# utiasASRL/dICP

Hardware: AMD Instinct MI355X
Metric: ICP cloud-iterations/sec (fwd+bwd), B=256x16384-pt clouds per GPU (higher is better)
Workload: dtype f32

## Files before the change

### dicp_amd/_lib.py

```python
import ctypes
import os
import subprocess
import threading

_HERE = os.path.dirname(os.path.abspath(__file__))
_ROOT = os.path.dirname(_HERE)
LIB_PATH = os.environ.get("DICP_HIP_LIB") or os.path.join(_HERE, "libdicp_hip.so")
SOURCES = [os.path.join(_HERE, "csrc", f) for f in ("dicp_kernels.hip", "knn_f16.hip", "dicp_call.hip", "normals.hip", "voxel.hip", "knn_points.hip", "fps.hip", "ball_query.hip", "knn_grid.hip", "group.hip", "inverse.hip", "knn_det.hip", "normals_det.hip", "filter.hip")]
HEADERS = ([os.path.join(_HERE, "csrc", f) for f in ("dicp_math.h", "dicp_common.h", "dicp_internal.h", "dicp_fill.h", "dicp_normals.h", "dicp_voxel.h", "dicp_topk.h", "dicp_fps.h", "dicp_ball.h", "dicp_gridknn.h", "kernels_grid.h", "kernels_grid_plan.h", "dicp_group.h", "dicp_group_launch.h", "dicp_inverse.h", "dicp_knn_det.h", "kernels_normals.h", "dicp_normals_det.h", "dicp_filter.h")]
           + [os.path.join(_HERE, "csrc", "kernels_%s.h" % f) for f in ("setup", "search", "setup_sort", "rows", "accumulate", "backward", "soft_svd", "host")]
           + [os.path.join(_ROOT, "include", "dicp_hip.h")])

F32, F64 = 0, 1
PT2PT, PT2PL = 0, 1
LOSS_NONE, LOSS_HUBER, LOSS_CAUCHY, LOSS_TRIM = 0, 1, 2, 3
KNN_AUTO, KNN_VALU, KNN_MFMA, KNN_SWEEP, KNN_GUMBEL = 0, 1, 2, 3, 4
FPS_AUTO, FPS_RESIDENT, FPS_STREAMED = 0, 1, 2
POOL_SUM, POOL_MEAN, POOL_MAX = 0, 1, 2
NACC_PAD, NBWD_PAD, KAB_SAVE = 32, 16, 40
PAIR_SHARDS = 64
ABI_VERSION = 11
_ERRORS = {1: "null pointer", 2: "bad shape/stride", 3: "unsupported dtype", 4: "bad enum value", 5: "misaligned buffer"}

vp, i32, i64, f64 = ctypes.c_void_p, ctypes.c_int32, ctypes.c_int64, ctypes.c_double


class WeightParams(ctypes.Structure):
    _fields_ = [("mode", i32), ("trim_on", i32), ("differentiable", i32), ("loss", i32),
                ("trim_dist", f64), ("tanh_k", f64), ("loss_delta", f64), ("match_thresh", f64)]


class StepIO(ctypes.Structure):
    _fields_ = [("partials", vp), ("nblk", i32), ("iter", i32), ("dim", i32), ("const_iter", i32),
                ("tolerance", f64), ("rows_per_point", i32), ("n", i32),
                ("pose_in", vp), ("pose_out", vp), ("delta", vp), ("delta_stride", i64),
                ("cost", vp), ("cost_prev", vp), ("cost_stride", i64), ("areg", vp), ("alive", vp), ("alive_out", vp),
                ("converged", vp), ("iterations", vp), ("matched_ratio", vp), ("n_start", vp),
                ("n_matched", vp), ("w_cur", vp), ("w_prev", vp), ("w_stride", i64), ("n_not_converged", vp),
                ("frame", vp), ("pose_search_out", vp), ("rmax", vp), ("dcum", vp), ("dcum_stride", i64), ("cert_cloud", vp),
                ("cert_qu", vp), ("cert_units", i32), ("glist_cap", i32), ("glist", vp), ("gcount", vp), ("cert_scount", vp), ("cert_slist", vp), ("w_copied", i32)]


class SearchBuffers(ctypes.Structure):
    _fields_ = [("knn_variant", i32), ("m_pad", i32), ("tgt4", vp), ("tperm", vp), ("qorder", vp), ("bucket", vp), ("brange", vp), ("nbkt", i32), ("pairs", vp), ("frame", vp), ("poses", vp),
                ("tgt_sorted", vp), ("tgt_sorted_stride", i32), ("gumbel", vp), ("first_done", i32), ("tgt_f16", vp), ("form", vp), ("form_default", i32), ("form_plan", vp)]


class CertBuffers(ctypes.Structure):
    _fields_ = [("q", vp), ("qu", vp), ("set", vp), ("count", vp), ("rmax", vp), ("dcum", vp), ("reset", i32), ("cloud", vp), ("nbr", vp), ("gdirty", vp), ("pend", vp), ("glist", vp),
                ("gcount", vp), ("slist", vp), ("scount", vp), ("cm", vp)]


class HistoryBuffers(ctypes.Structure):
    _fields_ = [("per_iter", i32), ("spos", vp), ("poses", vp), ("deltas", vp), ("costs", vp), ("areg", vp), ("alive", vp), ("idx", vp), ("w", vp), ("w_iter", i64), ("w_stride", i64),
                ("w_prev0", vp), ("spos_prev_chunk", vp), ("spos_floor", i32), ("spos_of", vp), ("spos_of_from", i32)]


class BwdBuffers(ctypes.Structure):
    _fields_ = [("spos_ref", vp), ("gts_far", vp), ("overwrite", i32), ("skip", vp), ("mref", vp), ("live", vp), ("skip_eps", f64), ("tail_from", i32), ("tail_partials", vp),
                ("tail_arrive", vp), ("det_far_row", vp), ("det_far_val", vp)]


class LoopBuffers(ctypes.Structure):
    _fields_ = [("abi", i32), ("src", vp), ("tgt", vp), ("w_init", vp), ("c", i32), ("K", i32), ("converged", vp), ("iterations", vp), ("matched_ratio", vp), ("n_start", vp), ("n_matched", vp),
                ("partials", vp), ("counters", vp), ("counters_host", vp), ("counters_tag", i32), ("events", vp), ("src_rows", vp), ("tgt_rows", vp),
                ("search", SearchBuffers), ("cert", CertBuffers), ("hist", HistoryBuffers), ("bwd", BwdBuffers)]

    def __init__(self, **kw):
        super().__init__(abi=ABI_VERSION)
        subs = (self, self.search, self.cert, self.hist, self.bwd)
        where = LoopBuffers._KW
        for k, v in kw.items():
            if v is not None:
                i, f = where[k]
                setattr(subs[i], f, v)


LoopBuffers._KW = dict([(f[0], (0, f[0])) for f in LoopBuffers._fields_[:-4]] +
                       [(g + "_" + f[0], (i + 1, f[0])) for i, (g, cls) in enumerate((("search", SearchBuffers), ("cert", CertBuffers), ("hist", HistoryBuffers), ("bwd", BwdBuffers)))
                        for f in cls._fields_])


class GumbelLoop(ctypes.Structure):
    _fields_ = [("U", vp), ("seeds", vp), ("eps", f64), ("tau", f64), ("ps_t", vp), ("nbr", vp), ("lse", vp), ("g_nbr", vp), ("g_ps", vp)]


MAX_SEGMENTS = 16
CERT_OFF_FOR_GOOD = 1 << 20


class SegmentPlan(ctypes.Structure):
    _fields_ = [("nseg", i32), ("k0", i32 * MAX_SEGMENTS), ("k1", i32 * MAX_SEGMENTS), ("new_order", i32 * MAX_SEGMENTS),
                ("cert_from", i32), ("pad0", i32), ("order", vp * MAX_SEGMENTS), ("keys", vp), ("cert_q", vp), ("cert_qu", vp), ("cert_count", vp), ("cert_cloud", vp), ("cert_set", vp),
                ("cert_nbr", vp), ("cert_gdirty", vp), ("cert_pend", vp), ("cert_cm", vp), ("cert_glist", vp), ("cert_gcount", vp), ("cert_slist", vp), ("cert_scount", vp)]


class Call(ctypes.Structure):
    _fields_ = [("src", vp), ("tgt", vp), ("T_init", vp), ("w0", vp), ("N", i32), ("n", i32), ("m", i32), ("c", i32), ("K", i32), ("dim", i32), ("need_grad", i32),
                ("n_resort", i32), ("resort", i32 * MAX_SEGMENTS), ("flags", i32), ("directions", i32), ("quantum", f64), ("tolerance", f64), ("workspace", vp), ("results", vp), ("T_out", vp), ("pc_out", vp)]


_sz = ctypes.c_size_t


class CallLayout(ctypes.Structure):
    _fields_ = ([(k, _sz) for k in ("total", "zeroed", "results_total", "results_zeroed", "T", "pc", "deltas", "weights", "costs", "converged", "iterations", "matched_ratio", "pairs", "n_matched", "counters",
                                    "poses", "poses_search", "alive", "areg", "n_start", "partials", "tgs4", "tperm", "bucket", "brange", "keys", "tgt_sorted", "scratch",
                                    "scratch_bytes", "frame", "pose_s", "orders", "spos")]
                + [("n_orders", i32), ("m_pad", i32), ("nblk", i32), ("pad0", i32)])


class CallGrads(ctypes.Structure):
    _fields_ = [("gT", vp), ("gsrc", vp), ("gtgt", vp), ("gT0", vp), ("gw", vp), ("workspace", vp), ("skip_eps", f64), ("tail_from", i32), ("pad0", i32), ("live_host", vp)]


class CallBackwardLayout(ctypes.Structure):
    _fields_ = ([(k, _sz) for k in ("total", "zeroed", "live", "arrive", "mref", "decisions", "far", "gpose", "gtmp", "src_s", "w_s", "gsrc_s", "gw_s", "slab", "gs", "gb",
                                    "partials", "tail_partials", "spos_ref")] + [("nblk_w", i32), ("pad0", i32)])


class LoopBackwardIn(ctypes.Structure):
    _fields_ = ([(k, vp) for k in ("src", "tgt_sorted", "w0", "tperm", "qorder", "spos", "poses", "deltas", "areg", "alive", "src_rows", "tgt_rows", "spos_of")]
                + [(k, i32) for k in ("N", "n", "m", "c", "K", "K_cap", "m_pad", "dim", "knn_variant", "spos_of_from")]
                + [(k, vp) for k in ("src_s", "w_s", "spos_ref")])


class KabschCall(ctypes.Structure):
    _fields_ = [("src", vp), ("tgt", vp), ("T_start", vp), ("w0", vp), ("N", i32), ("n", i32), ("m", i32), ("c", i32), ("K", i32), ("trim_on", i32), ("directions", i32), ("pad0", i32),
                ("trim_dist", f64), ("quantum", f64), ("tolerance", f64), ("workspace", vp), ("T_out", vp), ("pc_out", vp)]


class KabschCallLayout(ctypes.Structure):
    _fields_ = ([(k, _sz) for k in ("total", "zeroed", "costs", "iterations", "pairs", "counters", "frame", "keys", "tperm", "bucket", "brange", "tgs4", "scratch", "scratch_bytes",
                                    "pose", "pose_search", "pose_used", "partials", "save", "idx", "rows_live", "orders", "gpose", "gacc")] + [("m_pad", i32), ("nblk", i32)])


class KabschCallGrads(ctypes.Structure):
    _fields_ = [("gT", vp), ("gsrc", vp), ("gtgt", vp), ("gw", vp)]


CALL_FIRST_SEARCH, CALL_NO_SMALL_LOOP, CALL_NBKT = 1, 2, 1024


class KabschBuffers(ctypes.Structure):
    _fields_ = [("src", vp), ("tgt", vp), ("w_init", vp), ("c", i32), ("K", i32), ("knn_variant", i32), ("m_pad", i32), ("tgt4", vp), ("tperm", vp),
                ("qorder", vp), ("bucket", vp), ("brange", vp), ("nbkt", i32), ("pad0", i32), ("pairs", vp), ("frame", vp), ("pose", vp),
                ("pose_search", vp), ("pose_used", vp), ("idx", vp), ("partials", vp), ("save", vp), ("costs", vp), ("iterations", vp),
                ("rows_live", vp), ("tgt_rows", vp), ("counters", vp), ("tgt_f16", vp)]


_SIGNATURES = {
    "dicp_abi_version": ([], ctypes.c_int),
    "dicp_copy": ([vp, vp, ctypes.c_size_t, vp], ctypes.c_int),
    "dicp_zero": ([vp, ctypes.c_size_t, vp], ctypes.c_int),
    "dicp_padded_targets": ([i32], ctypes.c_int),
    "dicp_accumulate_blocks": ([i32], ctypes.c_int),
    "dicp_pack_target": ([i32, vp, i32, vp, vp, i32, i32, vp, i32, vp], ctypes.c_int),
    "dicp_search_frame": ([i32, vp, i32, vp, i32, i32, f64, i32, vp, vp, i32, vp, vp, vp], ctypes.c_int),
    "dicp_knn_f16_bytes": ([i32, i32], ctypes.c_size_t),
    "dicp_knn_f16_pack": ([vp, vp, i32, i32, i32, vp, vp], ctypes.c_int),
    "dicp_knn_f16_probe": ([vp, vp, vp, vp, vp, vp, i32, i32, i32, i32, vp, vp], ctypes.c_int),
    "dicp_knn": ([i32, vp, vp, vp, vp, vp, i32, i32, i32, i32, vp, i32, vp, vp], ctypes.c_int),
    "dicp_knn_sweep": ([i32, vp, vp, vp, vp, vp, vp, vp, i32, vp, vp, i32, i32, i32, i32, vp, vp, vp, i32, vp, vp, vp, i32, vp], ctypes.c_int),
    "dicp_window_blocks": ([i32, i32, i32], ctypes.c_int),
    "dicp_window_rows": ([i32], ctypes.c_int),
    "dicp_bwd_tail_max_blocks": ([i32], ctypes.c_int),
    "dicp_sweep_sort_scratch_bytes": ([i32, i32, i32], ctypes.c_size_t),
    "dicp_sweep_sort": ([i32, vp, i32, vp, vp, i32, i32, i32, vp, vp, i32, vp, vp, vp, ctypes.c_size_t, vp], ctypes.c_int),
    "dicp_sweep_build": ([i32, vp, i32, vp, vp, vp, i32, i32, i32, vp, vp, i32, vp], ctypes.c_int),
    "dicp_sweep_setup": ([i32, vp, i32, vp, i32, i32, i32, f64, i32, vp, vp, vp, i32, vp, vp, vp, ctypes.c_size_t, vp, vp, i32, vp, vp, i32, vp, vp, vp, vp], ctypes.c_int),
    "dicp_query_order": ([i32, vp, vp, vp, i32, i32, i32, vp, vp, vp, vp, i32, vp, i32, vp, vp, i32, vp, vp, vp], ctypes.c_int),
    "dicp_query_reorder": ([i32, vp, vp, vp, vp, vp, i32, i32, i32, vp, i32, vp, vp, i32, vp, vp, vp], ctypes.c_int),
    "dicp_query_keys": ([i32, vp, vp, i32, i32, vp, vp], ctypes.c_int),
    "dicp_loop_init": ([i32, vp, vp, ctypes.c_double, i32, i32, i32, vp, vp, vp, vp, vp, vp, vp, vp, i32, vp], ctypes.c_int),
    "dicp_search_pose": ([i32, vp, vp, i32, vp, vp], ctypes.c_int),
    "dicp_loop_finish": ([i32, vp, vp, vp, vp, i32, i32, vp, vp, vp, vp], ctypes.c_int),
    "dicp_accumulate_bwd_window": ([i32, ctypes.POINTER(WeightParams), vp, vp, i32, vp, vp, vp, vp, vp, vp, vp, vp, vp, i32, i32, i32, vp, vp, vp, vp, vp, i32, vp], ctypes.c_int),
    "dicp_resolve_matches": ([vp, vp, i32, vp, i32, i32, vp, vp], ctypes.c_int),
    "dicp_match_order_scratch_bytes": ([i32, i32, i32], ctypes.c_size_t),
    "dicp_match_order": ([i32, vp, vp, i32, i32, vp, ctypes.c_size_t, vp, vp], ctypes.c_int),
    "dicp_window_reduce": ([i32, vp, vp, vp, vp, vp, vp, i32, i32, i32, i32, i32, vp, i32, i32, vp], ctypes.c_int),
    "dicp_permute_add_rows": ([i32, vp, vp, i32, i32, i32, i32, i32, i32, vp, i32, i32, vp], ctypes.c_int),
    "dicp_pose_grad_in": ([i32, vp, vp, i32, vp], ctypes.c_int),
    "dicp_pose_grad_out": ([i32, vp, vp, i32, vp, i32, vp], ctypes.c_int),
    "dicp_permute_rows": ([i32, vp, vp, i32, i32, i32, i32, i32, i32, vp, i32, i32, vp], ctypes.c_int),
    "dicp_gather_rows": ([i32, vp, vp, i32, i32, i32, i32, vp, vp], ctypes.c_int),
    "dicp_scatter_add_rows": ([i32, vp, vp, i32, i32, i32, i32, vp, vp], ctypes.c_int),
    "dicp_pack_list": ([i32, vp, vp, vp, i32, i32, i32, vp, vp, vp], ctypes.c_int),
    "dicp_unpack_list": ([i32, vp, vp, vp, vp, i32, i32, i32, i32, vp], ctypes.c_int),
    "dicp_accumulate": ([i32, ctypes.POINTER(WeightParams), vp, vp, i32, vp, vp, vp, vp, vp, i32, i32, i32, vp, vp, i64, vp], ctypes.c_int),
    "dicp_step": ([i32, ctypes.POINTER(StepIO), i32, vp], ctypes.c_int),
    "dicp_icp_forward": ([i32, ctypes.POINTER(WeightParams), ctypes.POINTER(LoopBuffers), i32, i32, i32, i32, i32, f64, i32, i32, vp], ctypes.c_int),
    "dicp_icp_forward_plan": ([i32, ctypes.POINTER(WeightParams), ctypes.POINTER(LoopBuffers), ctypes.POINTER(SegmentPlan), i32, i32, i32, i32, i32, f64, vp], ctypes.c_int),
    "dicp_icp_backward": ([i32, ctypes.POINTER(WeightParams), ctypes.POINTER(LoopBuffers), i32, i32, i32, i32, vp, vp, i32, vp, vp, vp, vp, vp, vp, i32, i32, vp], ctypes.c_int),
    "dicp_step_bwd": ([i32, vp, vp, i32, i32, vp, vp, i64, vp, vp, vp, vp, i32, vp], ctypes.c_int),
    "dicp_accumulate_bwd": ([i32, ctypes.POINTER(WeightParams), vp, vp, i32, vp, vp, vp, vp, vp, vp, vp, i32, i32, i32, vp, vp, vp, vp, vp], ctypes.c_int),
    "dicp_gumbel_nn": ([i32, vp, vp, i32, vp, ctypes.c_uint32, f64, f64, i32, i32, i32, vp, vp, vp], ctypes.c_int),
    "dicp_gumbel_nn_bwd": ([i32, vp, vp, i32, vp, ctypes.c_uint32, f64, f64, vp, vp, vp, i32, i32, i32, vp, vp, vp], ctypes.c_int),
    "dicp_kabsch_accumulate": ([i32, vp, vp, i32, vp, vp, vp, i32, f64, vp, i32, i32, i32, vp, vp], ctypes.c_int),
    "dicp_kabsch_step": ([i32, vp, i32, vp, vp, vp, i32, vp], ctypes.c_int),
    "dicp_kabsch_step_bwd": ([i32, vp, vp, vp, i32, vp], ctypes.c_int),
    "dicp_kabsch_forward": ([i32, ctypes.POINTER(KabschBuffers), i32, i32, i32, i32, f64, i32, f64, i32, i32, vp], ctypes.c_int),
    "dicp_kabsch_bwd": ([i32, vp, vp, i32, vp, vp, vp, i32, f64, vp, vp, i32, i32, i32, vp, vp, vp, vp], ctypes.c_int),
    "dicp_transform_points": ([i32, vp, vp, vp, i32, i32, vp], ctypes.c_int),
    "dicp_transform_points_bwd": ([i32, vp, vp, vp, vp, vp, i32, i32, vp], ctypes.c_int),
    "dicp_loss_weight": ([i32, i32, i32, f64, f64, vp, i64, i32, vp, vp], ctypes.c_int),
    "dicp_loss_weight_bwd": ([i32, i32, i32, f64, f64, vp, vp, i64, i32, vp, vp], ctypes.c_int),
    "dicp_call_plan": ([i32, ctypes.POINTER(Call), ctypes.POINTER(CallLayout)], ctypes.c_int),
    "dicp_call_forward": ([i32, ctypes.POINTER(WeightParams), ctypes.POINTER(Call), vp], ctypes.c_int),
    "dicp_call_backward_plan": ([i32, ctypes.POINTER(WeightParams), ctypes.POINTER(Call), i32, i32, ctypes.POINTER(CallBackwardLayout)], ctypes.c_int),
    "dicp_call_backward": ([i32, ctypes.POINTER(WeightParams), ctypes.POINTER(Call), ctypes.POINTER(CallGrads), vp], ctypes.c_int),
    "dicp_loop_backward_plan": ([i32, ctypes.POINTER(WeightParams), ctypes.POINTER(LoopBackwardIn), i32, i32, ctypes.POINTER(CallBackwardLayout)], ctypes.c_int),
    "dicp_loop_backward": ([i32, ctypes.POINTER(WeightParams), ctypes.POINTER(LoopBackwardIn), ctypes.POINTER(CallGrads), vp], ctypes.c_int),
    "dicp_loop_backward_prepare": ([i32, ctypes.POINTER(LoopBackwardIn), vp, vp, vp, vp], ctypes.c_int),
    "dicp_kabsch_call_plan": ([i32, ctypes.POINTER(KabschCall), ctypes.POINTER(KabschCallLayout)], ctypes.c_int),
    "dicp_kabsch_call_forward": ([i32, ctypes.POINTER(KabschCall), vp], ctypes.c_int),
    "dicp_kabsch_call_backward": ([i32, ctypes.POINTER(KabschCall), ctypes.POINTER(KabschCallGrads), vp], ctypes.c_int),
    "dicp_normals_workspace_bytes": ([i32, i32, i32, i32, i32, i32], ctypes.c_size_t),
    "dicp_normals_forward": ([i32, vp, i32, vp, i32, i32, i32, vp, i32, vp, vp, vp, vp, ctypes.c_size_t, vp, vp], ctypes.c_int),
    "dicp_normals_backward": ([i32, vp, vp, vp, i32, vp, i32, i32, i32, i32, vp, vp, vp, ctypes.c_size_t, vp], ctypes.c_int),
    "dicp_normals_grid_workspace_bytes": ([i32, i32, i32, i32, i32, i32], ctypes.c_size_t),
    "dicp_normals_grid_forward": ([i32, vp, i32, vp, i32, i32, i32, vp, i32, vp, vp, vp, vp, ctypes.c_size_t, vp, vp, vp], ctypes.c_int),
    "dicp_normals_grid_backward": ([i32, vp, vp, vp, i32, i32, i32, i32, i32, vp, vp, vp, ctypes.c_size_t, vp], ctypes.c_int),
    "dicp_voxel_workspace_bytes": ([i32, i32, i32, i32], ctypes.c_size_t),
    "dicp_voxel_count": ([i32, vp, i32, vp, i32, i32, f64, f64, f64, vp, i32, i32, vp, vp, ctypes.c_size_t, vp], ctypes.c_int),
    "dicp_voxel_reduce": ([i32, vp, i32, i32, i32, i32, vp, ctypes.c_size_t, vp, vp, vp, vp], ctypes.c_int),
    "dicp_voxel_backward": ([i32, vp, vp, vp, i32, i32, i32, i32, vp, vp], ctypes.c_int),
    "dicp_knn_points_workspace_bytes": ([i32, i32, i32, i32, i32, i32], ctypes.c_size_t),
    "dicp_knn_points": ([i32, vp, vp, vp, i32, vp, vp, vp, vp, i32, i32, i32, vp, vp, vp, ctypes.c_size_t, vp, vp], ctypes.c_int),
    "dicp_knn_points_backward": ([i32, vp, vp, vp, vp, i32, i32, vp, vp, i32, i32, i32, i32, vp, vp, vp, vp, ctypes.c_size_t, vp], ctypes.c_int),
    "dicp_fps_geometry": ([i32, ctypes.POINTER(i32), ctypes.POINTER(i32), ctypes.POINTER(i32)], None),
    "dicp_fps_workspace_bytes": ([i32, i32, i32, i32, i32], ctypes.c_size_t),
    "dicp_fps_forward": ([i32, vp, i32, vp, vp, i32, i32, i32, i32, vp, vp, vp, vp, vp, ctypes.c_size_t, vp], ctypes.c_int),
    "dicp_fps_backward": ([i32, vp, vp, i32, i32, i32, i32, vp, vp], ctypes.c_int),
    "dicp_ball_grid_slots": ([i32], ctypes.c_int),
    "dicp_ball_plan_bytes": ([], ctypes.c_int),
    "dicp_ball_grid_build": ([i32, vp, i32, vp, i32, i32, vp, vp, vp, vp, vp, vp, vp], ctypes.c_int),
    "dicp_ball_query_workspace_bytes": ([i32, i32, i32, i32], ctypes.c_size_t),
    "dicp_ball_query": ([i32, vp, i32, i32, vp, vp, vp, vp, vp, vp, i32, i32, i32, vp, vp, vp, vp, ctypes.c_size_t, vp, vp], ctypes.c_int),
    "dicp_ball_query_backward": ([i32, vp, vp, i32, i32, vp, vp, i32, i32, i32, i32, vp, vp, vp, vp], ctypes.c_int),
    "dicp_knn_grid_build": ([i32, vp, i32, vp, i32, i32, vp, vp, vp, vp, vp], ctypes.c_int),
    "dicp_knn_grid_query": ([i32, vp, i32, i32, vp, vp, vp, vp, vp, vp, i32, i32, i32, vp, vp, vp, ctypes.c_size_t, vp, vp, vp], ctypes.c_int),
    "dicp_group_forward": ([i32, vp, vp, i32, vp, vp, i32, i32, i32, i32, i32, i32, vp, vp], ctypes.c_int),
    "dicp_group_backward": ([i32, vp, vp, i32, vp, i32, i32, i32, i32, i32, i32, vp, vp, vp], ctypes.c_int),
    "dicp_interpolate_forward": ([i32, vp, vp, i32, vp, vp, f64, i32, i32, i32, i32, i32, vp, vp], ctypes.c_int),
    "dicp_interpolate_backward": ([i32, vp, vp, vp, vp, i32, vp, vp, f64, i32, i32, i32, i32, i32, vp, vp, vp], ctypes.c_int),
    "dicp_pool_forward": ([i32, vp, vp, i32, vp, i32, i32, i32, i32, i32, i32, vp, vp, vp, vp], ctypes.c_int),
    "dicp_pool_backward": ([i32, vp, vp, i32, vp, i32, vp, vp, i32, i32, i32, i32, i32, vp, vp], ctypes.c_int),
    "dicp_invert_neighbors_workspace_bytes": ([i32, i32, i32, i32], ctypes.c_size_t),
    "dicp_invert_neighbors": ([vp, i32, vp, i32, i32, i32, i32, vp, vp, vp, ctypes.c_size_t, vp], ctypes.c_int),
    "dicp_group_backward_det": ([i32, vp, vp, i32, vp, i32, i32, i32, i32, i32, vp, vp, vp, vp], ctypes.c_int),
    "dicp_pool_backward_det": ([i32, vp, vp, i32, vp, i32, vp, vp, i32, i32, i32, i32, i32, vp, vp, vp, vp], ctypes.c_int),
    "dicp_interpolate_backward_det": ([i32, vp, vp, i32, vp, vp, f64, i32, i32, i32, i32, i32, vp, vp, vp, vp], ctypes.c_int),
    "dicp_knn_backward_y_det": ([i32, vp, vp, vp, vp, i32, i32, vp, i32, i32, i32, i32, vp, vp, vp, vp], ctypes.c_int),
    "dicp_normals_backward_records": ([i32, i32, vp, vp, vp, i32, vp, i32, i32, i32, i32, vp, ctypes.c_size_t, vp, vp, vp], ctypes.c_int),
    "dicp_normals_gather_det": ([i32, vp, vp, i32, vp, i32, i32, i32, i32, vp, vp, vp, vp], ctypes.c_int),
    "dicp_select_workspace_bytes": ([i32, i32], ctypes.c_size_t),
    "dicp_select_rows": ([i32, vp, i32, vp, vp, i32, i32, vp, vp, vp, vp, vp, ctypes.c_size_t, vp], ctypes.c_int),
    "dicp_select_rows_backward": ([i32, vp, vp, i32, i32, i32, vp, vp], ctypes.c_int),
    "dicp_outlier_workspace_bytes": ([i32, i32], ctypes.c_size_t),
    "dicp_outlier_stats": ([i32, vp, vp, vp, i32, i32, i32, f64, vp, vp, vp, vp, ctypes.c_size_t, vp], ctypes.c_int),
}
EXPORTS = tuple(_SIGNATURES)

_lib = None
_lock = threading.Lock()


FLAGS = ["-O3", "-std=c++17", "--offload-arch=gfx950", "-fPIC", "-ffp-contract=on", "-mllvm", "-amdgpu-mfma-vgpr-form", "-Wall", "-Wno-unused-function"]


def build(force=False, verbose=False):
    hdr_time = max(os.path.getmtime(p) for p in HEADERS + [os.path.abspath(__file__)])
    hipcc = os.environ.get("HIPCC", "/opt/rocm/bin/hipcc")
    objdir = os.path.join(_HERE, "csrc", "_obj")
    os.makedirs(objdir, exist_ok=True)
    jobs = []
    for src in SOURCES:
        obj = os.path.join(objdir, os.path.splitext(os.path.basename(src))[0] + ".o")
        if force or not os.path.exists(obj) or os.path.getmtime(obj) < max(os.path.getmtime(src), hdr_time):
            jobs.append((src, obj))
    objs = [os.path.join(objdir, os.path.splitext(os.path.basename(src))[0] + ".o") for src in SOURCES]
    if not jobs and os.path.exists(LIB_PATH) and os.path.getmtime(LIB_PATH) >= max(os.path.getmtime(o) for o in objs):
        return LIB_PATH

    def compile_one(job):
        cmd = [hipcc] + FLAGS + ["-I", os.path.join(_ROOT, "include"), "-c", "-o", job[1] + ".tmp", job[0]]
        if verbose:
            print(" ".join(cmd))
        subprocess.check_call(cmd)
        os.replace(job[1] + ".tmp", job[1])
    if jobs:
        from concurrent.futures import ThreadPoolExecutor
        with ThreadPoolExecutor(max_workers=min(len(jobs), 4)) as pool:
            list(pool.map(compile_one, jobs))
    cmd = [hipcc, "--offload-arch=gfx950", "-shared", "-fPIC", "-o", LIB_PATH + ".tmp"] + objs
    if verbose:
        print(" ".join(cmd))
    subprocess.check_call(cmd)
    os.replace(LIB_PATH + ".tmp", LIB_PATH)
    return LIB_PATH


def load():
    global _lib
    if _lib is not None:
        return _lib
    import torch
    with _lock:
        if _lib is None:
            if not os.path.exists(LIB_PATH):
                raise RuntimeError(
                    "dicp_amd: %s is missing -- build it with `python -c 'import __graft_entry__ as g; g.build()'` "
                    "(hipcc --offload-arch=gfx950).  There is no CPU fallback." % LIB_PATH)
            lib = ctypes.CDLL(LIB_PATH)
            for name, (args, res) in _SIGNATURES.items():
                fn = getattr(lib, name)
                fn.argtypes = args
                fn.restype = res
            if lib.dicp_abi_version() != ABI_VERSION:
                raise RuntimeError("dicp_amd: libdicp_hip.so ABI version mismatch; rebuild it")
            _lib = lib
    return _lib
# ... 20 lines not shown
```

### dicp_amd/_ops.py

```python
import os
import ctypes

import torch

from . import _lib

_DT = {torch.float32: _lib.F32, torch.float64: _lib.F64}
SWEEP_MIN_TARGETS = 2048
SWEEP_MIN_QUERIES = 256
F16_SWEEP = True
F16_SWEEP_MIN_QUERIES = 2 * 256 * 1024
F16_SWEEP_MIN_TARGETS = 16384
FORM_PLAN_ITERS = 6
FORM_TILES_MOVING = 32
F16_SWEEP_STATIC_TARGETS = 32768
F16_SWEEP_ADAPTIVE = os.environ.get("DICP_F16_ADAPTIVE", "1") != "0"
FORM_TILES = 12
SWEEP_MIN_PAIRS = 1e8


def auto_knn_kind(N, n, m):
    big = m >= SWEEP_MIN_TARGETS and n >= SWEEP_MIN_QUERIES and float(N) * n * m >= SWEEP_MIN_PAIRS
    return _lib.KNN_SWEEP if big else _lib.KNN_VALU
_LOSS = {None: _lib.LOSS_NONE, "huber": _lib.LOSS_HUBER, "cauchy": _lib.LOSS_CAUCHY, "trim": _lib.LOSS_TRIM}
# ... 19 lines not shown


def _stream():
    if _raw_stream is not None and _raw_device is not None:
        return ctypes.c_void_p(_raw_stream(_raw_device()))
    return ctypes.c_void_p(torch.cuda.current_stream().cuda_stream)


def _p(t):
    return ctypes.c_void_p(t.data_ptr()) if t is not None else None


def _workspace(nbytes, device):
    buf = torch.empty(nbytes + 256, dtype=torch.uint8, device=device)
    return buf[(-buf.data_ptr()) % 256:]


class _NoSwitch:
    def __enter__(self):
        return None

    def __exit__(self, *exc):
        return False


_NO_SWITCH = _NoSwitch()


def _on(device):
    if _raw_device is not None and device.index is not None and _raw_device() == device.index:
        return _NO_SWITCH
    return torch.cuda.device(device)


def padded_targets(m):
    return _lib.load().dicp_padded_targets(int(m))


def accumulate_blocks(n):
    return _lib.load().dicp_accumulate_blocks(int(n))


CENTER_QUANTUM = 16.0
FRAME_DIRECTIONS = True


def search_frame(tgt, quantum=None, tgt_rows=None, directions=None, src=None, T_init=None, src_rows=None):
    require_device(tgt, "search_frame")
    N, m, c = tgt.shape
    out = torch.empty((N, 12), dtype=tgt.dtype, device=tgt.device)
    with_q = src is not None and T_init is not None
    if with_q:
        src, T_init = src.contiguous(), T_init.contiguous()
    with _on(tgt.device):
        _lib.check(_lib.load().dicp_search_frame(_DT[tgt.dtype], _p(tgt), c, _p(tgt_rows), N, m, CENTER_QUANTUM if quantum is None else float(quantum),
                                                 int(FRAME_DIRECTIONS if directions is None else directions),
                                                 _p(src) if with_q else None, _p(src_rows) if with_q else None, int(src.shape[1]) if with_q else 0,
                                                 _p(T_init) if with_q else None, _p(out), _stream()), "dicp_search_frame")
    return out


def search_pose(pose, frame, N=None):
    if pose is None:
        if frame is not None:
            return frame.clone()
        pose = torch.zeros((N, 12))
        pose[:, 0] = pose[:, 4] = pose[:, 8] = 1.0
        return pose
    if frame is None:
        return pose
    n = pose.shape[0]
    Q, t = frame[:, :9].reshape(n, 3, 3), frame[:, 9:]
    out = torch.empty_like(pose)
    out[:, :9] = torch.matmul(Q, pose[:, :9].reshape(n, 3, 3)).reshape(n, 9)
    out[:, 9:] = torch.matmul(Q, pose[:, 9:, None]).squeeze(-1) + t
    return out


def pack_target(tgt, frame=None, tgt_rows=None):
    require_device(tgt, "pack_target")
    tgt = tgt.contiguous()
    N, m, c = tgt.shape
    m_pad = padded_targets(m)
    out = torch.empty((N, m_pad, 4), dtype=tgt.dtype, device=tgt.device)
    with _on(tgt.device):
        _lib.check(_lib.load().dicp_pack_target(_DT[tgt.dtype], _p(tgt), c, _p(frame), _p(tgt_rows), N, m, _p(out), m_pad, _stream()),
                   "dicp_pack_target")
    return out


def f16_image(tgt4, m, tgt_rows=None):
    require_device(tgt4, "f16_image")
    if tgt4.dtype != torch.float32:
        raise TypeError("dicp_amd.f16_image: the matrix-core search is float32 only")
    lib = _lib.load()
    N, m_pad, _ = tgt4.shape
    img = torch.empty((int(lib.dicp_knn_f16_bytes(N, m_pad)),), dtype=torch.uint8, device=tgt4.device)
    with _on(tgt4.device):
        _lib.check(lib.dicp_knn_f16_pack(_p(tgt4), _p(tgt_rows), N, int(m), m_pad, _p(img), _stream()), "dicp_knn_f16_pack")
    return img


def f16_counters(image, N, m_pad):
    m_img = (int(m_pad) + 511) // 512 * 512
    meta = image[N * m_img * 32:N * m_img * 32 + N * 320].view(torch.int32).view(N, 80)
    return int(meta[:, 6].sum().item()), int(meta[:, 7].sum().item())


def knn(src, pose, tgt4, m, variant=_lib.KNN_AUTO, out=None, src_rows=None, tgt_rows=None, image=None):
    require_device(src, "knn")
    N, n, _ = src.shape
    idx = out if out is not None else torch.empty((N, n), dtype=torch.int32, device=src.device)
    if (variant & 0xff) == _lib.KNN_MFMA and image is None and src.dtype == torch.float32:
        image = f16_image(tgt4, m, tgt_rows)
    with _on(src.device):
        _lib.check(_lib.load().dicp_knn(_DT[src.dtype], _p(src), _p(pose), _p(tgt4), _p(src_rows), _p(tgt_rows), N, n, m, tgt4.shape[1],
                                        _p(idx), variant, _p(image), _stream()), "dicp_knn")
    return idx


class SweepIndex:
    NBKT = 1024

    def __init__(self, tgt, sorted_rows=False, frame=None, tgt_rows=None, first_order=None, first_search=False, tally=True):
        require_device(tgt, "SweepIndex")
        tgt = tgt.contiguous()
        N, m, c = tgt.shape
        self.m = m
        self.frame, self.tgt_rows = frame, tgt_rows
        lib = _lib.load()
        dev, dt = tgt.device, tgt.dtype
        m_pad = lib.dicp_padded_targets(m)
        self.tgs4 = torch.empty((N, m_pad, 4), dtype=dt, device=dev)
        self.tperm = torch.empty((N, m_pad), dtype=torch.int32, device=dev)
        self.bucket = torch.empty((N, self.NBKT + 1), dtype=torch.int32, device=dev)
        self.brange = torch.empty((N, 2), dtype=dt, device=dev)
        self.keys = torch.empty((N, m_pad), dtype=dt, device=dev)
        self.row_stride = c
        self.tgt_s = torch.empty((N, m_pad, self.row_stride), dtype=dt, device=dev) if sorted_rows else None
        nbytes = int(lib.dicp_sweep_sort_scratch_bytes(_DT[dt], N, m_pad))
        scratch = torch.empty((nbytes,), dtype=torch.uint8, device=dev) if nbytes else None
        self.first = None
        self.pair_shards = torch.zeros((_lib.PAIR_SHARDS,), dtype=torch.int64, device=dev)
        self.img16 = None
        want_img = (bool(F16_SWEEP) and dt == torch.float32 and first_order is not None and float(N) * first_order[0].shape[1] >= F16_SWEEP_MIN_QUERIES
                    and m >= F16_SWEEP_MIN_TARGETS)
        self.form_default = int(m >= F16_SWEEP_MIN_TARGETS)
        self.form0 = None
        if first_order is not None:
            source, T_init, src_rows = first_order
            self.frame = torch.empty((N, 12), dtype=dt, device=dev)
            pose_s = torch.empty((N, 12), dtype=dt, device=dev)
            qorder = torch.empty((N, source.shape[1]), dtype=torch.int32, device=dev)
            with _on(dev):
                _lib.check(lib.dicp_sweep_setup(_DT[dt], _p(tgt), c, _p(tgt_rows), N, m, m_pad, CENTER_QUANTUM, int(FRAME_DIRECTIONS), _p(self.frame), _p(self.keys), _p(self.tperm),
                                                self.NBKT, _p(self.bucket), _p(self.brange), _p(scratch), nbytes, _p(self.tgs4), _p(self.tgt_s), self.row_stride,
                                                _p(source), _p(src_rows), source.shape[1], _p(T_init), _p(pose_s), _p(qorder), _stream()), "dicp_sweep_setup")
            if want_img:
                self.img16 = f16_image(self.tgs4, m, tgt_rows)
            spos0 = None
            if first_search:
                spos0 = torch.empty((N, source.shape[1]), dtype=torch.int32, device=dev)
                if tally and F16_SWEEP_ADAPTIVE and dt == torch.float32 and float(N) * source.shape[1] >= F16_SWEEP_MIN_QUERIES and bool(F16_SWEEP):
                    self.form0 = torch.zeros((N,), dtype=torch.int32, device=dev)
                with _on(dev):
                    _lib.check(lib.dicp_knn_sweep(_DT[dt], _p(source), _p(pose_s), _p(self.tgs4), _p(self.tperm), _p(qorder), _p(self.bucket), _p(self.brange), self.NBKT,
                                                  _p(src_rows), _p(tgt_rows), N, source.shape[1], m, m_pad, None, _p(spos0), _p(self.pair_shards), 0,
                                                  _p(self.img16) if (self.form_default or not F16_SWEEP_ADAPTIVE) else None, None, _p(self.form0), self.form_default, _stream()), "dicp_knn_sweep")
            self.first = (source, T_init, qorder, spos0)
            return
        with _on(dev):
            _lib.check(lib.dicp_sweep_sort(_DT[dt], _p(tgt), c, _p(frame), _p(tgt_rows), N, m, m_pad, _p(self.keys), _p(self.tperm), self.NBKT,
                                           _p(self.bucket), _p(self.brange), _p(scratch), nbytes, _stream()), "dicp_sweep_sort")
            _lib.check(lib.dicp_sweep_build(_DT[dt], _p(tgt), c, _p(frame), _p(tgt_rows), _p(self.tperm), N, m, m_pad,
                                            _p(self.tgs4), _p(self.tgt_s), self.row_stride, _stream()), "dicp_sweep_build")

    @property
    def pairs(self):
        return self.pair_shards.sum()

    def query_order(self, src, pose, exact=False, w=None, copies=False, reproducible=False, spos_prev=None, src_rows=None, pose_prev=None, order_prev=None):
        N, n, _ = src.shape
        lib = _lib.load()
        with _on(src.device):
            if not exact and pose is not None and pose_prev is not None and order_prev is not None and not copies and spos_prev is None:
                qorder = torch.empty((N, n), dtype=torch.int32, device=src.device)
                _lib.check(lib.dicp_query_reorder(_DT[src.dtype], _p(src), _p(pose), _p(pose_prev), _p(order_prev), _p(self.brange), self.NBKT, N, n, _p(qorder),
                                                  self.tgs4.shape[1], _p(self.keys), _p(self.bucket), self.m, _p(src_rows), _p(self.tgt_rows), _stream()), "dicp_query_reorder")
                return qorder
            if not exact:
                qorder = torch.empty((N, n), dtype=torch.int32, device=src.device)
                _lib.check(lib.dicp_query_order(_DT[src.dtype], _p(src), _p(pose), _p(self.brange), self.NBKT, N, n, _p(qorder),
                                                None, None, None, int(reproducible), _p(spos_prev), self.tgs4.shape[1],
                                                _p(self.keys), _p(self.bucket), self.m, _p(src_rows), _p(self.tgt_rows), _stream()),
                           "dicp_query_order")
                if copies:
                    return qorder, _gather_rows_raw(src, qorder), (_gather_rows_raw(w.unsqueeze(-1), qorder).squeeze(-1) if w is not None else None)
                return qorder
            assert src_rows is None, "exact query order: dense batches only (a test / tuning aid)"
            keys = torch.empty((N, n), dtype=src.dtype, device=src.device)
            _lib.check(lib.dicp_query_keys(_DT[src.dtype], _p(src), _p(pose), N, n, _p(keys), _stream()), "dicp_query_keys")
        qorder = torch.argsort(keys, dim=1).to(torch.int32)
        if copies:
            return qorder, _gather_rows_raw(src, qorder), (_gather_rows_raw(w.unsqueeze(-1), qorder).squeeze(-1) if w is not None else None)
        return qorder

    def make_image(self):
        if self.img16 is None:
            self.img16 = f16_image(self.tgs4, self.m, self.tgt_rows)
        return self.img16

    def knn(self, src, pose, qorder=None, out=None, cfg=0, spos=None, src_rows=None, mfma=False):
        N, n, _ = src.shape
        idx = out if out is not None else torch.empty((N, n), dtype=torch.int32, device=src.device)
        with _on(src.device):
            _lib.check(_lib.load().dicp_knn_sweep(_DT[src.dtype], _p(src), _p(pose), _p(self.tgs4), _p(self.tperm), _p(qorder),
                                                  _p(self.bucket), _p(self.brange), self.NBKT, _p(src_rows), _p(self.tgt_rows), N, n, self.m, self.tgs4.shape[1],
                                                  _p(idx), _p(spos), _p(self.pair_shards), cfg, _p(self.make_image()) if mfma else None, None, None, 1, _stream()), "dicp_knn_sweep")
        return idx


class _GatherRows(torch.autograd.Function):

    @staticmethod
    def forward(ctx, y, idx):
        N, m, c = y.shape
        n = idx.shape[1]
        out = torch.empty((N, n, c), dtype=y.dtype, device=y.device)
        with _on(y.device):
            _lib.check(_lib.load().dicp_gather_rows(_DT[y.dtype], _p(y), _p(idx), N, n, m, c, _p(out), _stream()), "dicp_gather_rows")
        ctx.save_for_backward(idx)
        ctx.shape = (N, m, c)
        return out

    @staticmethod
    def backward(ctx, gout):
        (idx,) = ctx.saved_tensors
        N, m, c = ctx.shape
        gout = gout.contiguous()
        gy = torch.zeros((N, m, c), dtype=gout.dtype, device=gout.device)
        with _on(gout.device):
            _lib.check(_lib.load().dicp_scatter_add_rows(_DT[gout.dtype], _p(gout), _p(idx), N, idx.shape[1], m, c, _p(gy), _stream()),
                       "dicp_scatter_add_rows")
        return gy, None


def gather_rows(y, idx):
    return _GatherRows.apply(y.contiguous(), idx)


def _gather_rows_raw(y, idx):
    y = y.contiguous()
    N, m, c = y.shape
    k = idx.shape[1]
    out = torch.empty((N, k, c), dtype=y.dtype, device=y.device)
    with _on(y.device):
        _lib.check(_lib.load().dicp_gather_rows(_DT[y.dtype], _p(y), _p(idx), N, k, m, c, _p(out), _stream()), "dicp_gather_rows")
    return out


class _PackList(torch.autograd.Function):

    @staticmethod
    def forward(ctx, cols, pad, *clouds):
        lib = _lib.load()
        N, dev, dt = len(clouds), clouds[0].device, clouds[0].dtype
        for t in clouds:
            if not (t.is_cuda and t.device == dev and t.dtype == dt and t.dim() == 2 and t.shape[1] >= cols and (t.shape[0] <= 1 or t.stride(1) == 1) and t.stride(0) >= t.shape[1]):
                raise ValueError("pack_list: every cloud must be a 2-D %s tensor on %s with unit column stride and at least %d columns" % (dt, dev, cols))
        lens = [int(t.shape[0]) for t in clouds]
        n_max = max(lens)
        meta = torch.tensor([t.data_ptr() for t in clouds] + lens + [int(t.stride(0)) for t in clouds], dtype=torch.int64).to(dev)
        lens_d, strides_d = meta[N:2 * N].to(torch.int32), meta[2 * N:].to(torch.int32)
        out = torch.empty((N, n_max, cols), dtype=dt, device=dev)
        with _on(dev):
            _lib.check(lib.dicp_pack_list(_DT[dt], _p(meta), _p(lens_d), _p(strides_d), N, n_max, int(cols), _p(out), _p(pad), _stream()), "dicp_pack_list")
        ctx.geom = (cols, n_max, lens, [int(t.shape[1]) for t in clouds], dt, dev)
        ctx.lens_d = lens_d
        return out

    @staticmethod
    def backward(ctx, gout):
        cols, n_max, lens, widths, dt, dev = ctx.geom
        lib = _lib.load()
        N, es = len(lens), torch.empty((), dtype=dt).element_size()
        sizes = [l * c for l, c in zip(lens, widths)]
        offs = [0]
        for sz in sizes:
            offs.append(offs[-1] + sz)
        flat = torch.empty((offs[-1],), dtype=dt, device=dev)
        meta = torch.tensor([flat.data_ptr() + o * es for o in offs[:-1]] + widths, dtype=torch.int64).to(dev)
        strides_d = meta[N:].to(torch.int32)
        g = gout.contiguous()
        with _on(dev):
            _lib.check(lib.dicp_unpack_list(_DT[dt], _p(g), _p(meta), _p(ctx.lens_d), _p(strides_d), N, n_max, int(cols), max(widths), _stream()), "dicp_unpack_list")
        grads = tuple(flat[offs[i]:offs[i + 1]].view(lens[i], widths[i]) if ctx.needs_input_grad[2 + i] else None for i in range(N))
        return (None, None) + grads


def packable(clouds, widths):
    first = clouds[0]
    if not isinstance(first, torch.Tensor) or not first.is_cuda or first.dtype not in _DT:
        return False
    return all(isinstance(t, torch.Tensor) and t.is_cuda and t.dim() == 2 and t.shape[0] > 0 and t.shape[1] in widths and t.dtype == first.dtype
               and t.device == first.device and t.stride(1) == 1 for t in clouds)


def pack_list(clouds, cols, pad=None):
    return _PackList.apply(int(cols), pad, *clouds)


class _GumbelNN(torch.autograd.Function):
# ... 276 lines not shown
```

### dicp_amd/csrc/dicp_internal.h

```cpp
#pragma once
#include <stddef.h>
#include <stdint.h>

namespace dicp_tu {

constexpr int KNN_F16_META = 80;
constexpr int KNN_F16_STAGE_ROWS = 512;
inline int knn_f16_image_rows(int m_pad) { return (m_pad + KNN_F16_STAGE_ROWS - 1) / KNN_F16_STAGE_ROWS * KNN_F16_STAGE_ROWS; }
inline size_t knn_f16_image_bytes(int N, int m_pad) { return (size_t)N * ((size_t)knn_f16_image_rows(m_pad) * 32 + KNN_F16_META * 4 + (size_t)knn_f16_image_rows(m_pad) / 64 * 8); }
inline size_t knn_f16_meta_offset(int N, int m_pad) { return (size_t)N * knn_f16_image_rows(m_pad) * 32; }
inline size_t knn_f16_edges_offset(int N, int m_pad) { return knn_f16_meta_offset(N, m_pad) + (size_t)N * KNN_F16_META * 4; }
int knn_f16_pack(const void* rows4, const int32_t* tgt_rows, int N, int m_full, int m_pad, void* image, void* stream);
int knn_f16_probe(const void* src, const void* pose, const void* tgt4, const void* image, const int32_t* src_rows, const int32_t* tgt_rows,
                  int N, int n, int m, int m_pad, float* out, void* stream);
int knn_f16_brute(const void* src, const void* pose, const void* tgt4, void* image, const int32_t* src_rows, const int32_t* tgt_rows,
                  int N, int n, int m, int m_pad, int32_t* idx, void* stream);

int knn_f16_sweep(const void* src, const void* pose, const void* tgs4, void* image, const int32_t* tperm, const int32_t* qorder, const int32_t* bucket,
                  const void* brange, int nbkt, const int32_t* src_rows, const int32_t* tgt_rows, int N, int n, int m, int m_pad, int32_t* idx, int32_t* spos,
                  unsigned long long* pairs, const int32_t* form_in, int32_t* form_out, int form_tiles, int form_default, void* ev0, void* ev1, void* stream);

}
```

### dicp_amd/csrc/dicp_kernels.hip

```cpp
#include <hip/hip_runtime.h>
#include <hip/hip_ext.h>
#include <stdint.h>

#include "dicp_common.h"
#include "dicp_internal.h"
#include "dicp_fill.h"

namespace {

#include "kernels_setup.h"
#include "kernels_search.h"
#include "kernels_setup_sort.h"
#include "kernels_rows.h"
#include "kernels_accumulate.h"
#include "kernels_backward.h"
#include "kernels_soft_svd.h"
#include "kernels_host.h"

}

extern "C" {

int dicp_abi_version(void) { return DICP_ABI_VERSION; }
int dicp_copy(void* dst, const void* src, size_t bytes, void* stream) {
    if (!dst || !src) return DICP_ERR_NULL;
    if ((((uintptr_t)dst | (uintptr_t)src | bytes) & 3) != 0) return DICP_ERR_ALIGN;
    return dicp_fill::copy(dst, src, bytes, (hipStream_t)stream);
}
int dicp_zero(void* dst, size_t bytes, void* stream) {
    if (!dst) return DICP_ERR_NULL;
    if ((((uintptr_t)dst | bytes) & 3) != 0) return DICP_ERR_ALIGN;
    return dicp_fill::zero(dst, bytes, (hipStream_t)stream);
}
int dicp_padded_targets(int m) { return m <= 0 ? 0 : ((m + KNN_PAD - 1) / KNN_PAD) * KNN_PAD; }
int dicp_accumulate_blocks(int n) { return n <= 0 ? 0 : (n + ACC_PTS - 1) / ACC_PTS; }
int dicp_search_frame(int dtype, const void* tgt, int c, const int32_t* tgt_rows, int N, int m, double quantum, int directions,
                      const void* src, const int32_t* src_rows, int n, const void* T_init, void* frame, void* stream) {
    if (!tgt || !frame) return DICP_ERR_NULL;
    if (bad_dtype(dtype)) return DICP_ERR_DTYPE;
    if (N <= 0 || m <= 0 || c < 3 || !(quantum >= 0.0) || (src && T_init && n <= 0)) return DICP_ERR_SHAPE;
    if (!src || !T_init) { src = nullptr; T_init = nullptr; }
    begin_launch();
    if (dtype == DICP_F32) search_frame_kernel<float><<<N, CC_THREADS, 0, (hipStream_t)stream>>>((const float*)tgt, c, m, tgt_rows, quantum, directions, (float*)frame, (const float*)src, n, src_rows, (const float*)T_init);
    else                   search_frame_kernel<double><<<N, CC_THREADS, 0, (hipStream_t)stream>>>((const double*)tgt, c, m, tgt_rows, quantum, directions, (double*)frame, (const double*)src, n, src_rows, (const double*)T_init);
    return launch_status();
}

int dicp_pack_target(int dtype, const void* tgt, int c, const void* frame, const int32_t* tgt_rows, int N, int m, void* tgt4, int m_pad, void* stream) {
    if (!tgt || !tgt4) return DICP_ERR_NULL;
    if (bad_dtype(dtype)) return DICP_ERR_DTYPE;
    if (N <= 0 || m <= 0 || (c != 3 && c != 6) || m_pad != dicp_padded_targets(m)) return DICP_ERR_SHAPE;
    if ((uintptr_t)tgt4 % (dtype == DICP_F32 ? 16 : 32)) return DICP_ERR_ALIGN;
    hipStream_t st = (hipStream_t)stream;
    begin_launch();
    const int bpc = (int)blocks_for((size_t)m_pad);
    const unsigned g = grid_for(N, bpc);
    if (dtype == DICP_F32) pack_kernel<float><<<g, BLOCK, 0, st>>>((const float*)tgt, N, m, c, (float4*)tgt4, m_pad, bpc, (const float*)frame, tgt_rows);
    else                   pack_kernel<double><<<g, BLOCK, 0, st>>>((const double*)tgt, N, m, c, (double4*)tgt4, m_pad, bpc, (const double*)frame, tgt_rows);
    return launch_status();
}

size_t dicp_sweep_sort_scratch_bytes(int dtype, int N, int m_pad) {
    if (N <= 0 || m_pad <= 0 || (dtype == DICP_F32 && m_pad <= RS_MAX)) return 0;
    const size_t S = ((size_t)m_pad + GS_CHUNK - 1) / GS_CHUNK, passes = dtype == DICP_F32 ? 4 : 8;
    return (size_t)N * 2 * m_pad * ((dtype == DICP_F32 ? 4 : 8) + sizeof(int32_t)) + 256 + (S <= GS_MAX_CHUNKS ? passes * (size_t)N * S * S * 256 * sizeof(int32_t) : 0);
}

int dicp_sweep_sort(int dtype, const void* tgt, int c, const void* frame, const int32_t* tgt_rows, int N, int m, int m_pad, void* keys_sorted,
                    int32_t* tperm, int nbkt, int32_t* bucket, void* brange, void* scratch, size_t scratch_bytes, void* stream) {
    if (!tgt || !keys_sorted || !tperm || (bucket && !brange)) return DICP_ERR_NULL;
    if (bucket && nbkt <= 0) return DICP_ERR_SHAPE;
    if (bad_dtype(dtype)) return DICP_ERR_DTYPE;
    if (N <= 0 || m <= 0 || (c != 3 && c != 6) || m_pad != dicp_padded_targets(m)) return DICP_ERR_SHAPE;
    hipStream_t st = (hipStream_t)stream;
    if (dtype == DICP_F32 && m_pad <= RS_MAX) {
        begin_launch();
        sort_keys_kernel<<<N, RS_THREADS, 0, st>>>((const float*)tgt, c, N, m, m_pad, (float*)keys_sorted, tperm, nbkt, bucket, (float*)brange, (const float*)frame, tgt_rows);
        return launch_status();
    }
    if (!scratch || scratch_bytes < dicp_sweep_sort_scratch_bytes(dtype, N, m_pad)) return DICP_ERR_NULL;
    begin_launch();
    void* kb = (void*)(((uintptr_t)scratch + 15) & ~(uintptr_t)15);
    const int S = (m_pad + GS_CHUNK - 1) / GS_CHUNK;
    const bool several = S >= 2 && S <= GS_MAX_CHUNKS && (size_t)N * S <= 0x7fffffffu;
#define DICP_BIGSORT(T, KT) do { \
        int32_t* ib = (int32_t*)((KT*)kb + (size_t)N * 2 * m_pad); \
        int32_t* hist = ib + (size_t)N * 2 * m_pad; \
        if (several) { \
            constexpr int PASSES = (int)sizeof(KT); \
            sort_big_keys_kernel<T><<<N * S, GS_THREADS, 0, st>>>((const T*)tgt, c, m, m_pad, S, (const T*)frame, tgt_rows, (KT*)kb, ib, hist, N); \
            for (int p = 0; p + 1 < PASSES; ++p) sort_big_pass_kernel<T, false><<<N * S, GS_THREADS, 0, st>>>(p, m_pad, S, (KT*)kb, ib, hist, N, (T*)keys_sorted, tperm); \
            sort_big_pass_kernel<T, true><<<N * S, GS_THREADS, 0, st>>>(PASSES - 1, m_pad, S, (KT*)kb, ib, hist, N, (T*)keys_sorted, tperm); \
        } else sort_keys_big_kernel<T><<<N, GS_THREADS, 0, st>>>((const T*)tgt, c, m, m_pad, (const T*)frame, tgt_rows, (T*)keys_sorted, tperm, (KT*)kb, ib); \
        if (bucket) sweep_buckets_kernel<T><<<N, BLOCK, 0, st>>>((const T*)keys_sorted, N, m, m_pad, nbkt, bucket, (T*)brange, tgt_rows); } while (0)
    if (dtype == DICP_F32) DICP_BIGSORT(float, unsigned); else DICP_BIGSORT(double, unsigned long long);
#undef DICP_BIGSORT
    return launch_status();
}

int dicp_sweep_build(int dtype, const void* tgt, int c, const void* frame, const int32_t* tgt_rows, const int32_t* tperm, int N, int m, int m_pad,
                     void* tgs4, void* tgt_s, int tgt_s_stride, void* stream) {
    if (!tgt || !tgs4 || !tperm) return DICP_ERR_NULL;
    if (bad_dtype(dtype)) return DICP_ERR_DTYPE;
    if (N <= 0 || m <= 0 || (c != 3 && c != 6) || m_pad != dicp_padded_targets(m) || (tgt_s && tgt_s_stride < c)) return DICP_ERR_SHAPE;
    if ((uintptr_t)tgs4 % (dtype == DICP_F32 ? 16 : 32)) return DICP_ERR_ALIGN;
    hipStream_t st = (hipStream_t)stream;
    begin_launch();
    const int bpc = (m_pad + BLOCK * 4 - 1) / (BLOCK * 4);
    const unsigned g = grid_for(N, bpc);
    if (dtype == DICP_F32) sweep_rows_kernel<float><<<g, BLOCK, 0, st>>>((const float*)tgt, tgt_rows, N, m, c, m_pad, bpc, (float4*)tgs4, tperm, (float*)tgt_s, tgt_s_stride, (const float*)frame);
    else                   sweep_rows_kernel<double><<<g, BLOCK, 0, st>>>((const double*)tgt, tgt_rows, N, m, c, m_pad, bpc, (double4*)tgs4, tperm, (double*)tgt_s, tgt_s_stride, (const double*)frame);
    return launch_status();
}

int dicp_sweep_setup(int dtype, const void* tgt, int c, const int32_t* tgt_rows, int N, int m, int m_pad, double quantum, int directions,
                     void* frame, void* keys_sorted, int32_t* tperm, int nbkt, int32_t* bucket, void* brange, void* scratch, size_t scratch_bytes,
                     void* tgs4, void* tgt_s, int tgt_s_stride,
                     const void* src, const int32_t* src_rows, int n, const void* T_init, void* pose_search0, int32_t* qorder0, void* stream) {
    if (!frame) return DICP_ERR_NULL;
    int rc = dicp_search_frame(dtype, tgt, c, tgt_rows, N, m, quantum, directions, src, src_rows, n, T_init, frame, stream);
    if (!rc) rc = dicp_sweep_sort(dtype, tgt, c, frame, tgt_rows, N, m, m_pad, keys_sorted, tperm, nbkt, bucket, brange, scratch, scratch_bytes, stream);
    if (!rc) rc = dicp_sweep_build(dtype, tgt, c, frame, tgt_rows, tperm, N, m, m_pad, tgs4, tgt_s, tgt_s_stride, stream);
    if (!rc && T_init && pose_search0 && qorder0) {
        if (!src || n <= 0) return DICP_ERR_NULL;
        rc = dicp_search_pose(dtype, T_init, frame, N, pose_search0, stream);
        if (!rc) rc = dicp_query_order(dtype, src, pose_search0, brange, nbkt, N, n, qorder0, nullptr, nullptr, nullptr, 0, nullptr, m_pad, keys_sorted, bucket, m,
                                       src_rows, tgt_rows, stream);
    }
    return rc;
}

int dicp_query_keys(int dtype, const void* src, const void* pose, int N, int n, void* keys, void* stream) {
    if (!src || !keys) return DICP_ERR_NULL;
    if (bad_dtype(dtype)) return DICP_ERR_DTYPE;
    if (N <= 0 || n <= 0) return DICP_ERR_SHAPE;
    hipStream_t st = (hipStream_t)stream;
    begin_launch();
    const int bpc = (int)blocks_for((size_t)n);
    const unsigned g = grid_for(N, bpc);
    if (dtype == DICP_F32) query_keys_kernel<float><<<g, BLOCK, 0, st>>>((const float*)src, (const float*)pose, N, n, bpc, (float*)keys);
    else                   query_keys_kernel<double><<<g, BLOCK, 0, st>>>((const double*)src, (const double*)pose, N, n, bpc, (double*)keys);
    return launch_status();
}

static int query_order_go(int dtype, const void* src, const void* pose, const void* brange, int nbkt, int N, int n, int32_t* qorder,
                          const void* w, void* src_s, void* w_s, int reproducible, const int32_t* spos_prev, int m_pad,
                          const void* skeys, const int32_t* bucket, int m, const int32_t* src_rows, const int32_t* tgt_rows, const void* pose_prev, const int32_t* order_prev, void* stream);
int dicp_query_order(int dtype, const void* src, const void* pose, const void* brange, int nbkt, int N, int n, int32_t* qorder,
                     const void* w, void* src_s, void* w_s, int reproducible, const int32_t* spos_prev, int m_pad,
                     const void* skeys, const int32_t* bucket, int m, const int32_t* src_rows, const int32_t* tgt_rows, void* stream) {
    return query_order_go(dtype, src, pose, brange, nbkt, N, n, qorder, w, src_s, w_s, reproducible, spos_prev, m_pad, skeys, bucket, m, src_rows, tgt_rows, nullptr, nullptr, stream);
}
int dicp_query_reorder(int dtype, const void* src, const void* pose, const void* pose_prev, const int32_t* order_prev, const void* brange, int nbkt, int N, int n,
                       int32_t* qorder, int m_pad, const void* skeys, const int32_t* bucket, int m, const int32_t* src_rows, const int32_t* tgt_rows, void* stream) {
    if (!pose || !pose_prev || !order_prev || order_prev == qorder) return DICP_ERR_NULL;
    return query_order_go(dtype, src, pose, brange, nbkt, N, n, qorder, nullptr, nullptr, nullptr, 0, nullptr, m_pad, skeys, bucket, m, src_rows, tgt_rows, pose_prev, order_prev, stream);
}
static int query_order_go(int dtype, const void* src, const void* pose, const void* brange, int nbkt, int N, int n, int32_t* qorder,
                          const void* w, void* src_s, void* w_s, int reproducible, const int32_t* spos_prev, int m_pad,
                          const void* skeys, const int32_t* bucket, int m, const int32_t* src_rows, const int32_t* tgt_rows, const void* pose_prev, const int32_t* order_prev, void* stream) {
    if (!src || !brange || !qorder || (w_s && !w)) return DICP_ERR_NULL;
    if (bad_dtype(dtype)) return DICP_ERR_DTYPE;
    if (N <= 0 || n <= 0 || nbkt <= 0 || ((spos_prev || skeys) && m_pad <= 0) || (skeys && (m <= 0 || m > m_pad))) return DICP_ERR_SHAPE;
    hipStream_t st = (hipStream_t)stream;
    begin_launch();
#define DICP_QO(T, S) query_order_kernel<T, S><<<N, QO_THREADS, 0, st>>>((const T*)src, (const T*)pose, (const T*)brange, nbkt, N, n, qorder, \
        (const T*)w, (T*)src_s, (T*)w_s, reproducible, spos_prev, m_pad, (const T*)skeys, 1, m, bucket, src_rows, tgt_rows, (const T*)pose_prev, order_prev)
    if (dtype == DICP_F32) { if (n <= 16384) DICP_QO(float, 16384); else DICP_QO(float, 65536); }
    else                   { if (n <= 16384) DICP_QO(double, 16384); else DICP_QO(double, 65536); }
#undef DICP_QO
    return launch_status();
}

int dicp_loop_init(int dtype, const void* T_init, const void* w0, double thresh, int rows, int N, int n,
                   void* pose0, void* alive0, void* n_start, const void* frame, void* pose_search0,
                   const void* src, void* rmax, void* dcum, int dcum_stride, void* stream) {
    if (!T_init || !pose0 || !alive0 || !n_start || (rmax && (!src || !dcum))) return DICP_ERR_NULL;
    if (bad_dtype(dtype)) return DICP_ERR_DTYPE;
    if (N <= 0 || n <= 0 || (rows != 1 && rows != 3) || (rmax && dcum_stride < 2)) return DICP_ERR_SHAPE;
    hipStream_t st = (hipStream_t)stream;
    begin_launch();
    if (dtype == DICP_F32) loop_init_kernel<float><<<N, LI_THREADS, 0, st>>>((const float*)T_init, (const float*)w0, (float)thresh, rows, n, (float*)pose0, (float*)alive0, (float*)n_start, (const float*)frame, (float*)pose_search0, (const float*)src, (float*)rmax, (float*)dcum, dcum_stride);
    else                   loop_init_kernel<double><<<N, LI_THREADS, 0, st>>>((const double*)T_init, (const double*)w0, thresh, rows, n, (double*)pose0, (double*)alive0, (double*)n_start, (const double*)frame, (double*)pose_search0, (const double*)src, (double*)rmax, (double*)dcum, dcum_stride);
    return launch_status();
}

int dicp_search_pose(int dtype, const void* T_init, const void* frame, int N, void* pose_search, void* stream) {
    if (!T_init || !pose_search) return DICP_ERR_NULL;
    if (bad_dtype(dtype)) return DICP_ERR_DTYPE;
    if (N <= 0) return DICP_ERR_SHAPE;
    begin_launch();
    const unsigned g = (unsigned)((N * 12 + BLOCK - 1) / BLOCK);
    if (dtype == DICP_F32) search_pose_kernel<float><<<g, BLOCK, 0, (hipStream_t)stream>>>((const float*)T_init, (const float*)frame, N, (float*)pose_search);
    else                   search_pose_kernel<double><<<g, BLOCK, 0, (hipStream_t)stream>>>((const double*)T_init, (const double*)frame, N, (double*)pose_search);
    return launch_status();
}

int dicp_loop_finish(int dtype, const void* pose_K, const void* alive_K, const void* n_start, const void* n_matched, int K, int N,
                     void* iterations, void* matched_ratio, void* T_out, void* stream) {
    if (!pose_K || !alive_K || !n_start || !n_matched || !iterations || !matched_ratio || !T_out) return DICP_ERR_NULL;
    if (bad_dtype(dtype)) return DICP_ERR_DTYPE;
    if (N <= 0 || K < 0) return DICP_ERR_SHAPE;
    hipStream_t st = (hipStream_t)stream;
    begin_launch();
    const unsigned g = blocks_for((size_t)N);
    if (dtype == DICP_F32) loop_finish_kernel<float><<<g, BLOCK, 0, st>>>((const float*)pose_K, (const float*)alive_K, (const float*)n_start, (const float*)n_matched, K, N, (float*)iterations, (float*)matched_ratio, (float*)T_out);
    else                   loop_finish_kernel<double><<<g, BLOCK, 0, st>>>((const double*)pose_K, (const double*)alive_K, (const double*)n_start, (const double*)n_matched, K, N, (double*)iterations, (double*)matched_ratio, (double*)T_out);
    return launch_status();
}

int dicp_pose_grad_in(int dtype, const void* gT, double* gpose, int N, void* stream) {
    if (!gpose) return DICP_ERR_NULL;
    if (bad_dtype(dtype)) return DICP_ERR_DTYPE;
    if (N <= 0) return DICP_ERR_SHAPE;
    hipStream_t st = (hipStream_t)stream;
    begin_launch();
    const unsigned g = blocks_for((size_t)N * 12);
    if (dtype == DICP_F32) pose_grad_in_kernel<float><<<g, BLOCK, 0, st>>>((const float*)gT, gpose, N);
    else                   pose_grad_in_kernel<double><<<g, BLOCK, 0, st>>>((const double*)gT, gpose, N);
    return launch_status();
}

int dicp_pose_grad_out(int dtype, const double* gpose, const void* bwd_partials, int nblk, void* gT0, int N, void* stream) {
    if (!gpose || !gT0) return DICP_ERR_NULL;
    if (bad_dtype(dtype)) return DICP_ERR_DTYPE;
    if (N <= 0 || (bwd_partials && nblk <= 0)) return DICP_ERR_SHAPE;
    hipStream_t st = (hipStream_t)stream;
    begin_launch();
    const unsigned g = blocks_for((size_t)N * 16);
    if (dtype == DICP_F32) pose_grad_out_kernel<float><<<g, BLOCK, 0, st>>>(gpose, (const float*)bwd_partials, nblk, (float*)gT0, N);
    else                   pose_grad_out_kernel<double><<<g, BLOCK, 0, st>>>(gpose, (const double*)bwd_partials, nblk, (double*)gT0, N);
    return launch_status();
}

int dicp_knn_f16_probe(const void* src, const void* pose, const void* tgt4, const void* f16_image, const int32_t* src_rows, const int32_t* tgt_rows,
                       int N, int n, int m, int m_pad, float* out, void* stream) {
    return dicp_tu::knn_f16_probe(src, pose, tgt4, f16_image, src_rows, tgt_rows, N, n, m, m_pad, out, stream);
}
size_t dicp_knn_f16_bytes(int N, int m_pad) { return (N <= 0 || m_pad <= 0) ? 0 : dicp_tu::knn_f16_image_bytes(N, m_pad); }
int dicp_knn_f16_pack(const void* tgt4, const int32_t* tgt_rows, int N, int m, int m_pad, void* image, void* stream) {
    return dicp_tu::knn_f16_pack(tgt4, tgt_rows, N, m, m_pad, image, stream);
}

int dicp_knn(int dtype, const void* src, const void* pose, const void* tgt4, const int32_t* src_rows, const int32_t* tgt_rows,
             int N, int n, int m, int m_pad, int32_t* idx, int variant, const void* f16_image, void* stream) {
    if (!src || !tgt4 || !idx) return DICP_ERR_NULL;
    if (bad_dtype(dtype)) return DICP_ERR_DTYPE;
    if (N <= 0 || n <= 0 || m <= 0 || m_pad != dicp_padded_targets(m)) return DICP_ERR_SHAPE;
    const int kind = variant & 0xff, cfg = (variant >> 8) & 0xff;
    if (kind < DICP_KNN_AUTO || kind > DICP_KNN_MFMA || (variant >> 16)) return DICP_ERR_ENUM;
    if (kind == DICP_KNN_MFMA && dtype != DICP_F32) return DICP_ERR_DTYPE;
    if ((uintptr_t)tgt4 % (dtype == DICP_F32 ? 16 : 32)) return DICP_ERR_ALIGN;
    hipStream_t st = (hipStream_t)stream;
    begin_launch();
    const Rows rw{src_rows, tgt_rows};
    if (kind == DICP_KNN_MFMA) {
        if (!f16_image) return DICP_ERR_NULL;
        return dicp_tu::knn_f16_brute(src, pose, tgt4, const_cast<void*>(f16_image), src_rows, tgt_rows, N, n, m, m_pad, idx, stream);
    }
    if (dtype == DICP_F32) return knn_valu_launch<float>(cfg, src, pose, tgt4, N, n, m, m_pad, idx, rw, st);
    return knn_valu_launch<double>(cfg, src, pose, tgt4, N, n, m, m_pad, idx, rw, st);
}

static int sweep_queries_per_lane(int cfg) { return cfg == 2 ? 2 : ((cfg == 1 || cfg == 4) ? 1 : 0); }
static int sweep_auto_cfg(int N, int n) { return ((long)N * n >= 2L * BLOCK * 1024) ? SWEEP_CFG_BIG : 4; }

static int guard_list_cap(int N, int n) { return (N > 2 ? N : 2) * ((n + WAVE - 1) / WAVE); }

struct CertArgs {
    void* q; void* qu; const void* dcum; int dstride; int k; int32_t* count; bool guard; int32_t* cloud; void* set;
    int32_t* cm; int32_t* pend; int32_t* gdirty;
    int32_t* slist; int32_t* scount;
    const int32_t* glist; const int32_t* gcount; int glist_cap;
};

struct FormArgs { const int32_t* in; int32_t* out; int dflt; };
static int sweep_launch(int dtype, const void* src, const void* pose, const void* tgs4, const int32_t* tperm,
                        const int32_t* qorder, const int32_t* bucket, const void* brange, int nbkt,
                        int N, int n, int m, int m_pad, int32_t* idx, int32_t* spos, unsigned long long* pairs, int cfg, Rows rw, hipStream_t st,
                        CertArgs ca = CertArgs{}, const void* f16_image = nullptr, FormArgs fa = FormArgs{nullptr, nullptr, 0}) {
    hipEvent_t ev0, ev1;
// ... 864 lines not shown
```

### dicp_amd/csrc/kernels_setup.h

```cpp
template <typename T> __device__ __forceinline__ T big_v();
template <> __device__ __forceinline__ float  big_v<float>()  { return 3.402823466e+38f; }
template <> __device__ __forceinline__ double big_v<double>() { return 1.7976931348623157e+308; }

template <typename T>
__device__ __forceinline__ bool frame_is_translation(const T* __restrict__ F) {
    return F[0] == T(1) && F[4] == T(1) && F[8] == T(1) && F[1] == T(0) && F[2] == T(0) && F[3] == T(0) && F[5] == T(0) && F[6] == T(0) && F[7] == T(0);
}
template <typename T>
__device__ __forceinline__ void frame_apply(const T* __restrict__ F, const T* y, T* out) {
    if (!F) { out[0] = y[0]; out[1] = y[1]; out[2] = y[2]; return; }
    if (frame_is_translation(F)) { out[0] = y[0] + F[9]; out[1] = y[1] + F[10]; out[2] = y[2] + F[11]; return; }
#pragma unroll
    for (int k = 0; k < 3; ++k) out[k] = fma_t(F[3 * k], y[0], fma_t(F[3 * k + 1], y[1], fma_t(F[3 * k + 2], y[2], F[9 + k])));
}
template <typename T>
__device__ __forceinline__ T frame_pose_entry(const T* __restrict__ F, const T* pose , int e) {
    if (!F) return pose[e];
    if (frame_is_translation(F)) return e < 9 ? pose[e] : pose[e] + F[e];
    if (e < 9) { const int i = e / 3, j = e - 3 * i; return fma_t(F[3 * i], pose[j], fma_t(F[3 * i + 1], pose[3 + j], F[3 * i + 2] * pose[6 + j])); }
    const int i = e - 9;
    return fma_t(F[3 * i], pose[9], fma_t(F[3 * i + 1], pose[10], fma_t(F[3 * i + 2], pose[11], F[9 + i])));
}

template <typename T>
__device__ __forceinline__ typename V4<T>::type pack_row(const T* __restrict__ y, const T* __restrict__ frame = nullptr) {
    typename V4<T>::type v;
    T q[3];
    frame_apply(frame, y, q);
    v.x = q[0]; v.y = q[1]; v.z = q[2];
    v.w = T(0.5) * fma_t(v.z, v.z, fma_t(v.y, v.y, v.x * v.x));
    return v;
}

constexpr int CC_THREADS = 1024;
constexpr int CC_SAMPLE = CC_THREADS;
constexpr int SF_DIRS = 6;
__device__ __forceinline__ unsigned sortable_bits(float x);
constexpr int SF_QUERIES = CC_THREADS / 4;
template <typename T>
__global__ __launch_bounds__(CC_THREADS) void search_frame_kernel(const T* __restrict__ tgt, int c, int m, const int32_t* __restrict__ tgt_rows,
                                                                  double quantum, int directions, T* __restrict__ frame,
                                                                  const T* __restrict__ src, int n, const int32_t* __restrict__ src_rows, const T* __restrict__ T_init) {
    const double QS[SF_DIRS][9] = {
        {1, 0, 0, 0, 1, 0, 0, 0, 1}, {0, 1, 0, 0, 0, 1, 1, 0, 0}, {0, 0, 1, 1, 0, 0, 0, 1, 0},
        {0.6, 0.64, 0.48, 0.72953720414008516, -0.68394112888132985, 0, 0.32829174186303833, 0.35017785798724088, -0.87726848797845247},
        {0.6, -0.64, 0.48, -0.72953720414008516, -0.68394112888132985, 0, 0.32829174186303833, -0.35017785798724088, -0.87726848797845247},
        {0.48, 0.6, -0.64, 0, -0.72953720414008516, -0.68394112888132985, -0.87726848797845247, 0.32829174186303833, -0.35017785798724088}};
    __shared__ int hist[3][256];
    __shared__ unsigned sel_prefix[3];
    __shared__ int sel_want[3];
    __shared__ int dhist[SF_DIRS][256];
    __shared__ float s_ctr[3], s_ext[CC_THREADS / WAVE], s_cnt[CC_THREADS / WAVE];
    __shared__ int s_cost[SF_DIRS];
    __shared__ float4 s_t[CC_SAMPLE];
    __shared__ int s_cum[SF_DIRS][256 + 1];
    const int cloud = blockIdx.x, tid = threadIdx.x, lane = tid & (WAVE - 1), wave = tid >> 6;
    const T* __restrict__ rows = tgt + (size_t)cloud * m * c;
    const int mc = max(rows_of(tgt_rows, cloud, m), 1);
    const int step = (mc + CC_SAMPLE - 1) / CC_SAMPLE, ms = (mc + step - 1) / step;
    const bool on = tid < ms;
    unsigned key[3] = {0u, 0u, 0u};
    float pt[3] = {0.f, 0.f, 0.f};
    if (on) {
        const T* r = rows + (size_t)tid * step * c;
        pt[0] = (float)r[0]; pt[1] = (float)r[1]; pt[2] = (float)r[2];
        key[0] = sortable_bits(pt[0]); key[1] = sortable_bits(pt[1]); key[2] = sortable_bits(pt[2]);
    }
    if (tid < 3) { sel_prefix[tid] = 0u; sel_want[tid] = (ms - 1) / 2; }
    unsigned mask = 0u;
    for (int pass = 3; pass >= 0; --pass) {
        for (int d = tid; d < 3 * 256; d += CC_THREADS) (&hist[0][0])[d] = 0;
        __syncthreads();
        if (on) {
#pragma unroll
            for (int a = 0; a < 3; ++a)
                if ((key[a] & mask) == sel_prefix[a]) atomicAdd(&hist[a][(key[a] >> (8 * pass)) & 255u], 1);
        }
        __syncthreads();
        if (wave < 3) {
            const int a = wave, want = sel_want[a];
            const int h0 = hist[a][4 * lane], h1 = hist[a][4 * lane + 1], h2 = hist[a][4 * lane + 2], h3 = hist[a][4 * lane + 3];
            int incl = h0 + h1 + h2 + h3;
            const int own = incl;
#pragma unroll
            for (int off = 1; off < WAVE; off <<= 1) { const int o = __shfl_up(incl, off); if (lane >= off) incl += o; }
            const unsigned long long over = __ballot(incl > want);
            const int L = over ? __ffsll((long long)over) - 1 : WAVE - 1;
            if (lane == L) {
                int w = want - (incl - own), d = 0;
                if (w >= h0) { w -= h0; d = 1; if (w >= h1) { w -= h1; d = 2; if (w >= h2) { w -= h2; d = 3; } } }
                sel_want[a] = w;
                sel_prefix[a] |= (unsigned)(4 * lane + d) << (8 * pass);
            }
        }
        mask |= 0xffu << (8 * pass);
        __syncthreads();
    }
    if (tid < 3) {
        unsigned u = sel_prefix[tid];
        u ^= (u >> 31) ? 0x80000000u : 0xffffffffu;
        double v = (double)__uint_as_float(u);
        v = quantum > 0.0 ? rint(v / quantum) * quantum : v;
        s_ctr[tid] = (v == v && fabs(v) < 1e30) ? (float)(T)v : 0.f;
    }
    for (int d = tid; d < SF_DIRS * 256; d += CC_THREADS) (&dhist[0][0])[d] = 0;
    __syncthreads();
    const float dx = pt[0] - s_ctr[0], dy = pt[1] - s_ctr[1], dz = pt[2] - s_ctr[2];
    const bool fin = on && fabsf(dx) < 1e30f && fabsf(dy) < 1e30f && fabsf(dz) < 1e30f;
    const float dev = fin ? fmaxf(fabsf(dx), fmaxf(fabsf(dy), fabsf(dz))) : 0.f;
    float dsum = dev, dcnt = fin ? 1.f : 0.f;
#pragma unroll
    for (int off = WAVE / 2; off > 0; off >>= 1) { dsum += __shfl_xor(dsum, off); dcnt += __shfl_xor(dcnt, off); }
    if (lane == 0) { s_ext[wave] = dsum; s_cnt[wave] = dcnt; }
    __syncthreads();
    float mean_dev = 0.f, cnt_all = 0.f;
    for (int w = 0; w < CC_THREADS / WAVE; ++w) { mean_dev += s_ext[w]; cnt_all += s_cnt[w]; }
    mean_dev = cnt_all > 0.f ? mean_dev / cnt_all : 0.f;
    __syncthreads();
    float ext = (fin && dev <= 32.f * mean_dev) ? dev : 0.f;
#pragma unroll
    for (int off = WAVE / 2; off > 0; off >>= 1) ext = fmaxf(ext, __shfl_xor(ext, off));
    if (lane == 0) s_ext[wave] = ext;
    __syncthreads();
    float R2 = 0.f;
    for (int w = 0; w < CC_THREADS / WAVE; ++w) R2 = fmaxf(R2, s_ext[w]);
    R2 *= 1.7321f;
    int best = 0;
    if (directions && R2 > 0.f) {
        if (fin) {
            const float scale = 128.f / R2;
#pragma unroll
            for (int j = 0; j < SF_DIRS; ++j) {
                const float k = (float)QS[j][0] * dx + (float)QS[j][1] * dy + (float)QS[j][2] * dz;
                const int bin = min(max((int)((k + R2) * scale), 0), 255);
                atomicAdd(&dhist[j][bin], 1);
            }
        }
        const bool with_queries = src != nullptr && T_init != nullptr && n > 0;
        if (with_queries) s_t[tid] = fin ? make_float4(dx, dy, dz, 0.f) : make_float4(1e18f, 1e18f, 1e18f, 0.f);
        __syncthreads();
        if (wave < SF_DIRS) {
            const int h0 = dhist[wave][4 * lane], h1 = dhist[wave][4 * lane + 1], h2 = dhist[wave][4 * lane + 2], h3 = dhist[wave][4 * lane + 3];
            int cst = h0 * h0 + h1 * h1 + h2 * h2 + h3 * h3;
#pragma unroll
            for (int off = WAVE / 2; off > 0; off >>= 1) cst += __shfl_xor(cst, off);
            if (lane == 0) s_cost[wave] = with_queries ? 0 : cst;
            if (with_queries) {
                int incl = h0 + h1 + h2 + h3;
                const int own = incl;
#pragma unroll
                for (int off = 1; off < WAVE; off <<= 1) { const int o = __shfl_up(incl, off); if (lane >= off) incl += o; }
                const int ex = incl - own;
                s_cum[wave][4 * lane] = ex; s_cum[wave][4 * lane + 1] = ex + h0; s_cum[wave][4 * lane + 2] = ex + h0 + h1; s_cum[wave][4 * lane + 3] = ex + h0 + h1 + h2;
                if (lane == WAVE - 1) s_cum[wave][256] = incl;
            }
        }
        __syncthreads();
        if (with_queries) {
            const int nc = rows_of(src_rows, cloud, n);
            const int qstep = max((nc + SF_QUERIES - 1) / SF_QUERIES, 1), nq = (nc + qstep - 1) / qstep;
            const int qid = tid >> 2, part = tid & 3;
            bool qon = qid < nq;
            float qx = 0.f, qy = 0.f, qz = 0.f;
            if (qon) {
                const T* p = src + ((size_t)cloud * n + (size_t)qid * qstep) * 3;
                const T* M = T_init + (size_t)cloud * 16;
                const float p0 = (float)p[0], p1 = (float)p[1], p2 = (float)p[2];
                qx = (float)M[0] * p0 + (float)M[1] * p1 + (float)M[2] * p2 + (float)M[3] - s_ctr[0];
                qy = (float)M[4] * p0 + (float)M[5] * p1 + (float)M[6] * p2 + (float)M[7] - s_ctr[1];
                qz = (float)M[8] * p0 + (float)M[9] * p1 + (float)M[10] * p2 + (float)M[11] - s_ctr[2];
                qon = fabsf(qx) < 1e18f && fabsf(qy) < 1e18f && fabsf(qz) < 1e18f;
            }
            float d2 = 3e38f;
            if (qon) {
                float da = 3e38f, db = 3e38f, dc = 3e38f, dd = 3e38f;
                int t = part;
                for (; t + 12 < ms; t += 16) {
                    const float4 a = s_t[t], b = s_t[t + 4], c4 = s_t[t + 8], e4 = s_t[t + 12];
                    da = fminf(da, (a.x - qx) * (a.x - qx) + (a.y - qy) * (a.y - qy) + (a.z - qz) * (a.z - qz));
                    db = fminf(db, (b.x - qx) * (b.x - qx) + (b.y - qy) * (b.y - qy) + (b.z - qz) * (b.z - qz));
                    dc = fminf(dc, (c4.x - qx) * (c4.x - qx) + (c4.y - qy) * (c4.y - qy) + (c4.z - qz) * (c4.z - qz));
                    dd = fminf(dd, (e4.x - qx) * (e4.x - qx) + (e4.y - qy) * (e4.y - qy) + (e4.z - qz) * (e4.z - qz));
                }
                for (; t < ms; t += 4) { const float4 a = s_t[t]; da = fminf(da, (a.x - qx) * (a.x - qx) + (a.y - qy) * (a.y - qy) + (a.z - qz) * (a.z - qz)); }
                d2 = fminf(fminf(da, db), fminf(dc, dd));
            }
            d2 = fminf(d2, __shfl_xor(d2, 1));
            d2 = fminf(d2, __shfl_xor(d2, 2));
            if (qon && d2 < 1e30f) {
                const float d = sqrtf(d2), scale = 128.f / R2;
#pragma unroll
                for (int j = 0; j < SF_DIRS; ++j) {
                    if ((j & 3) != part) continue;
                    const float k = (float)QS[j][0] * qx + (float)QS[j][1] * qy + (float)QS[j][2] * qz;
                    const int lo = min(max((int)((k - d + R2) * scale), 0), 255), hi = min(max((int)((k + d + R2) * scale), 0), 255);
                    atomicAdd(&s_cost[j], s_cum[j][hi + 1] - s_cum[j][lo]);
                }
            }
            __syncthreads();
        }
        for (int j = 1; j < SF_DIRS; ++j) if (s_cost[j] < s_cost[best]) best = j;
        if (!(5 * (long long)s_cost[best] < 4 * (long long)s_cost[0])) best = 0;
    }
    if (tid < 12) {
        T* F = frame + (size_t)cloud * 12;
        if (tid < 9) F[tid] = (T)QS[best][tid];
        else {
            const int i = tid - 9;
            const T cx = (T)s_ctr[0], cy = (T)s_ctr[1], cz = (T)s_ctr[2];
            F[tid] = best == 0 ? -(i == 0 ? cx : (i == 1 ? cy : cz))
                               : -fma_t((T)QS[best][3 * i], cx, fma_t((T)QS[best][3 * i + 1], cy, (T)QS[best][3 * i + 2] * cz));
        }
    }
}

template <typename T>
__global__ __launch_bounds__(BLOCK) void pack_kernel(const T* __restrict__ tgt, int N, int m, int c,
                                                     typename V4<T>::type* __restrict__ out, int m_pad, int bpc,
                                                     const T* __restrict__ frame, const int32_t* __restrict__ tgt_rows) {
    int b, blk;
    if (!decode_block(bpc, N, b, blk)) return;
    const int j = blk * BLOCK + threadIdx.x;
    if (j >= m_pad) return;
    typename V4<T>::type v;
    if (j < rows_of(tgt_rows, b, m)) v = pack_row<T>(tgt + ((size_t)b * m + j) * c, frame ? frame + (size_t)b * 12 : nullptr);
    else { v.x = v.y = v.z = T(0); v.w = inf_v<T>(); }
    out[(size_t)b * m_pad + j] = v;
}

template <typename T>
__global__ __launch_bounds__(BLOCK) void sweep_rows_kernel(const T* __restrict__ tgt, const int32_t* __restrict__ tgt_rows, int N, int m, int c,
                                                           int m_pad, int bpc, typename V4<T>::type* __restrict__ tgs4, const int32_t* __restrict__ tperm,
                                                           T* __restrict__ tgt_s , int rs ,
                                                           const T* __restrict__ frame ) {
    constexpr int U = 4;
    int b, blk;
    if (!decode_block(bpc, N, b, blk)) return;
    const int s0 = blk * (BLOCK * U) + threadIdx.x;
    const int mc = rows_of(tgt_rows, b, m);
    {
        int j[U];
        T y[U][6];
#pragma unroll
        for (int u = 0; u < U; ++u) {
            const size_t at = (size_t)b * m_pad + min(s0 + u * BLOCK, m_pad - 1);
            j[u] = tperm[at];
        }
        const bool full = tgt_s && c == 6;
#pragma unroll
        for (int u = 0; u < U; ++u) {
            const T* yp = tgt + ((size_t)b * m + (j[u] >= 0 && j[u] < mc ? j[u] : 0)) * c;
            y[u][0] = yp[0]; y[u][1] = yp[1]; y[u][2] = yp[2];
            if (full) { y[u][3] = yp[3]; y[u][4] = yp[4]; y[u][5] = yp[5]; }
        }
#pragma unroll
        for (int u = 0; u < U; ++u) {
            const int sl = s0 + u * BLOCK;
            if (sl >= m_pad) continue;
            typename V4<T>::type v;
            if (j[u] >= 0 && j[u] < mc) v = pack_row<T>(y[u], frame ? frame + (size_t)b * 12 : nullptr);
            else { v.x = big_v<T>(); v.y = v.z = T(0); v.w = inf_v<T>(); }
            tgs4[(size_t)b * m_pad + sl] = v;
            if (tgt_s) {
                T* o = tgt_s + ((size_t)b * m_pad + sl) * rs;
                o[0] = y[u][0]; o[1] = y[u][1]; o[2] = y[u][2];
                if (full) { o[3] = y[u][3]; o[4] = y[u][4]; o[5] = y[u][5]; }
                for (int k = c; k < rs; ++k) o[k] = T(0);
            }
        }
    }
}

template <typename T>
__global__ __launch_bounds__(BLOCK) void sweep_buckets_kernel(const T* __restrict__ keys , int N, int m_full, int m_pad,
                                                              int nbkt, int32_t* __restrict__ bucket, T* __restrict__ brange, const int32_t* __restrict__ tgt_rows) {
    const int cloud = blockIdx.x;
    const int m = max(rows_of(tgt_rows, cloud, m_full), 1);
    const T* __restrict__ xs = keys + (size_t)cloud * m_pad;
    const T xlo = xs[0], span = xs[m - 1] - xlo;
    for (int b = threadIdx.x; b <= nbkt; b += BLOCK) {
        const T edge = fma_t(T(b), span / T(nbkt), xlo);
        int lo = 0, hi = m;
        while (lo < hi) { const int mid = (lo + hi) >> 1; if (xs[mid] < edge) lo = mid + 1; else hi = mid; }
        bucket[(size_t)cloud * (nbkt + 1) + b] = lo;
    }
    if (threadIdx.x == 0) {
        brange[(size_t)cloud * 2] = xlo;
        brange[(size_t)cloud * 2 + 1] = span > T(0) ? T(nbkt) / span : T(0);
    }
}

constexpr int RS_THREADS = 1024, RS_PER = 16, RS_MAX = RS_THREADS * RS_PER;
__device__ __forceinline__ unsigned sortable_bits(float x) {
    unsigned u = __float_as_uint(x + 0.0f);
    u ^= (u >> 31) ? 0xffffffffu : 0x80000000u;
    return x != x ? 0xffffffffu : u;
}
__global__ __launch_bounds__(RS_THREADS) void sort_keys_kernel(const float* __restrict__ tgt, int c, int N, int m_full, int m_pad,
                                                               float* __restrict__ keys_sorted, int32_t* __restrict__ tperm,
                                                               int nbkt, int32_t* __restrict__ bucket, float* __restrict__ brange,
                                                               const float* __restrict__ frame, const int32_t* __restrict__ tgt_rows) {
    __shared__ unsigned skey[RS_MAX];
    __shared__ unsigned short sidx[RS_MAX];
    __shared__ int cnt[RS_THREADS / WAVE][256];
    __shared__ int tot[256];
    const int cloud = blockIdx.x, tid = threadIdx.x, lane = tid & (WAVE - 1), wave = tid >> 6;
    const float* __restrict__ rows = tgt + (size_t)cloud * m_full * c;
    const int m = rows_of(tgt_rows, cloud, m_full);
    unsigned key[RS_PER];
    unsigned short idx[RS_PER];
#pragma unroll
    for (int e = 0; e < RS_PER; ++e) {
        const int pos = wave * (WAVE * RS_PER) + e * WAVE + lane;
        unsigned u = 0xffffffffu;
        if (pos < m) { float q[3]; frame_apply<float>(frame ? frame + (size_t)cloud * 12 : nullptr, rows + (size_t)pos * c, q); u = sortable_bits(q[0]); }
        key[e] = u;
        idx[e] = (unsigned short)pos;
    }
    for (int pass = 0; pass < 4; ++pass) {
        const int shift = pass * 8;
        for (int d = lane; d < 256; d += WAVE) cnt[wave][d] = 0;
        __builtin_amdgcn_wave_barrier();
        int rank[RS_PER];
#pragma unroll
        for (int e = 0; e < RS_PER; ++e) {
            const unsigned d = (key[e] >> shift) & 0xffu;
            unsigned long long same = ~0ull;
#pragma unroll
            for (int b = 0; b < 8; ++b) {
                const unsigned long long bal = __ballot((d >> b) & 1u);
                same &= ((d >> b) & 1u) ? bal : ~bal;
            }
            const int below = __builtin_amdgcn_mbcnt_hi((unsigned)(same >> 32), __builtin_amdgcn_mbcnt_lo((unsigned)same, 0u));
            const int base = cnt[wave][d];
            __builtin_amdgcn_wave_barrier();
            if (below == 0) cnt[wave][d] = base + __popcll(same);
            __builtin_amdgcn_wave_barrier();
            rank[e] = base + below;
        }
        __syncthreads();
        if (tid < 256) {
            int s = 0;
            for (int w = 0; w < RS_THREADS / WAVE; ++w) { const int v = cnt[w][tid]; cnt[w][tid] = s; s += v; }
            tot[tid] = s;
        }
        __syncthreads();
        if (tid < WAVE) {
            int v[4], s = 0;
#pragma unroll
            for (int k = 0; k < 4; ++k) { v[k] = tot[lane * 4 + k]; s += v[k]; }
            int inc = s;
#pragma unroll
            for (int off = 1; off < WAVE; off <<= 1) { const int o = __shfl_up(inc, off); if (lane >= off) inc += o; }
            int run = inc - s;
#pragma unroll
            for (int k = 0; k < 4; ++k) { tot[lane * 4 + k] = run; run += v[k]; }
        }
        __syncthreads();
#pragma unroll
        for (int e = 0; e < RS_PER; ++e) {
            const unsigned d = (key[e] >> shift) & 0xffu;
            const int pos = tot[d] + cnt[wave][d] + rank[e];
            skey[pos] = key[e];
            sidx[pos] = idx[e];
        }
        __syncthreads();
#pragma unroll
        for (int e = 0; e < RS_PER; ++e) {
            const int pos = wave * (WAVE * RS_PER) + e * WAVE + lane;
            key[e] = skey[pos];
            idx[e] = sidx[pos];
        }
        __syncthreads();
    }
#pragma unroll
    for (int e = 0; e < RS_PER; ++e) {
        const int pos = wave * (WAVE * RS_PER) + e * WAVE + lane;
        if (pos < m_pad) {
            unsigned u = key[e];
            u ^= (u >> 31) ? 0x80000000u : 0xffffffffu;
            keys_sorted[(size_t)cloud * m_pad + pos] = __uint_as_float(u);
            tperm[(size_t)cloud * m_pad + pos] = (int32_t)idx[e];
        }
    }
    if (bucket) {
        auto key_at = [&](int i) { unsigned u = skey[i]; u ^= (u >> 31) ? 0x80000000u : 0xffffffffu; return __uint_as_float(u); };
        const float xlo = key_at(0), span = key_at(max(m, 1) - 1) - xlo;
        for (int b = tid; b <= nbkt; b += RS_THREADS) {
            const unsigned edge = sortable_bits(fma_t(float(b), span / float(nbkt), xlo));
            int lo = 0, hi = m;
            while (lo < hi) { const int mid = (lo + hi) >> 1; if (skey[mid] < edge) lo = mid + 1; else hi = mid; }
            bucket[(size_t)cloud * (nbkt + 1) + b] = lo;
        }
        if (tid == 0) {
            brange[(size_t)cloud * 2] = xlo;
            brange[(size_t)cloud * 2 + 1] = span > 0.f ? float(nbkt) / span : 0.f;
        }
    }
}

template <typename T>
__global__ __launch_bounds__(BLOCK) void query_keys_kernel(const T* __restrict__ src, const T* __restrict__ pose, int N, int n, int bpc,
                                                           T* __restrict__ keys) {
    int b, blk;
    if (!decode_block(bpc, N, b, blk)) return;
    const int i = blk * BLOCK + threadIdx.x;
    if (i >= n) return;
    {
        const size_t t = (size_t)b * n + i;
        const T* p = src + t * 3;
        T x = p[0];
        if (pose) {
            const T* q = pose + (size_t)b * 12;
            x = fma_t(q[0], p[0], fma_t(q[1], p[1], fma_t(q[2], p[2], q[9])));
        }
        keys[t] = x;
    }
}

constexpr int QO_THREADS = 1024;
constexpr int QO_BUCKETS = 2048;
constexpr int QO_KEYS = 16384;
constexpr int QO_TABLE = 1024;
constexpr int QO_SIDE = 256;
constexpr int QO_MID = QO_BUCKETS - 2 * QO_SIDE;
__device__ __forceinline__ int qo_side_bucket(float dist_scaled) { return (int)fminf(fmaxf(dist_scaled, 0.f), (float)(QO_SIDE - 1)); }
template <typename T, int QO_STAGE>
__global__ __launch_bounds__(QO_THREADS) void query_order_kernel(const T* __restrict__ src, const T* __restrict__ pose,
                                                                 const T* __restrict__ brange, int nbkt_range, int N, int n_full,
                                                                 int32_t* __restrict__ qorder, const T* __restrict__ w,
                                                                 T* __restrict__ src_s, T* __restrict__ w_s, int reproducible,
                                                                 const int32_t* __restrict__ spos_prev, int m_pad,
                                                                 const T* __restrict__ skeys, int kstride, int mt_full, const int32_t* __restrict__ table,
                                                                 const int32_t* __restrict__ src_rows, const int32_t* __restrict__ tgt_rows,
                                                                 const T* __restrict__ pose_prev = nullptr, const int32_t* __restrict__ order_prev = nullptr) {
    __shared__ int cnt[QO_BUCKETS];
    __shared__ int s_same;
    __shared__ int wsum[QO_THREADS / WAVE];
    __shared__ unsigned short stage[QO_STAGE];
    __shared__ float lkeys[QO_STAGE <= 16384 ? QO_KEYS : 1];
    __shared__ int ltab[QO_STAGE <= 16384 ? QO_TABLE + 1 : 1];
    const int cloud = blockIdx.x, tid = threadIdx.x;
    const int n = rows_of(src_rows, cloud, n_full), mt = max(rows_of(tgt_rows, cloud, mt_full), 1);
    src += (size_t)cloud * (n_full - n) * 3;
    if (w) w += (size_t)cloud * (n_full - n);
    if (spos_prev) spos_prev += (size_t)cloud * (n_full - n);
    qorder += (size_t)cloud * (n_full - n);
    if (src_s) src_s += (size_t)cloud * (n_full - n) * 3;
    if (w_s) w_s += (size_t)cloud * (n_full - n);
    for (int i = n + tid; i < n_full; i += QO_THREADS) {
        qorder[(size_t)cloud * n + i] = i;
        if (src_s) { const T* p = src + ((size_t)cloud * n + i) * 3; T* o = src_s + ((size_t)cloud * n + i) * 3; o[0] = p[0]; o[1] = p[1]; o[2] = p[2]; }
        if (w_s) w_s[(size_t)cloud * n + i] = w[(size_t)cloud * n + i];
    }
    if (n <= 0) return;
    if (pose && pose_prev && order_prev && !src_s && !w_s) {
        if (tid == 0) {
            const T* a = pose + (size_t)cloud * 12;
            const T* b = pose_prev + (size_t)cloud * 12;
            float dc = 0.f, dr = 0.f;
#pragma unroll
            for (int e = 0; e < 9; ++e) { const float d = (float)(a[e] - b[e]); dc += d * d; }
#pragma unroll
            for (int e = 9; e < 12; ++e) { const float d = (float)(a[e] - b[e]); dr += d * d; }
            const float x0 = (float)brange[(size_t)cloud * 2], ts = (float)brange[(size_t)cloud * 2 + 1];
            const float span = ts > 0.f ? (float)nbkt_range / ts : 0.f;
            const float moved = sqrtf(dc) * 1.7321f * fmaxf(fabsf(x0), fabsf(x0 + span)) + sqrtf(dr);
            s_same = (moved * (float)n < 0.1f * span * (float)(2 * WAVE)) ? 1 : 0;
        }
        __syncthreads();
        if (s_same) {
            const int32_t* op = order_prev + (size_t)cloud * (n_full - n);
            for (int i = tid; i < n; i += QO_THREADS) qorder[(size_t)cloud * n + i] = op[(size_t)cloud * n + i];
            return;
        }
    }
    for (int b = tid; b < QO_BUCKETS; b += QO_THREADS) cnt[b] = 0;
    T q[4] = {T(1), T(0), T(0), T(0)};
    if (pose) { const T* pp = pose + (size_t)cloud * 12; q[0] = pp[0]; q[1] = pp[1]; q[2] = pp[2]; q[3] = pp[9]; }
    const T xlo = brange[(size_t)cloud * 2];
    const T tscale = brange[(size_t)cloud * 2 + 1];
    const T scale = tscale * (T(QO_MID) / T(nbkt_range));
    const bool ranked = QO_STAGE <= 16384 && skeys && table && !spos_prev && mt <= QO_KEYS && nbkt_range <= QO_TABLE;
    if (ranked) {
        const T* __restrict__ keys = skeys + (size_t)cloud * m_pad * kstride;
        for (int j = tid; j < mt; j += QO_THREADS) lkeys[j] = (float)keys[(size_t)j * kstride];
        for (int j = tid; j <= nbkt_range; j += QO_THREADS) ltab[j] = table[(size_t)cloud * (nbkt_range + 1) + j];
    }
    const float span_w = tscale > T(0) ? (float)(T(nbkt_range) / tscale) : 0.f;
    const float side_w = span_w > 0.f ? (float)QO_SIDE / span_w : 0.f;
    auto bucket_of = [&](int i) {
        if (spos_prev) {
            const int sp = spos_prev[(size_t)cloud * n + i];
            return sp < 0 ? QO_BUCKETS - 1 : (int)(((long)min(sp, m_pad - 1) * QO_BUCKETS) / m_pad);
        }
        const T* p = src + ((size_t)cloud * n + i) * 3;
        const T x = fma_t(q[0], p[0], fma_t(q[1], p[1], fma_t(q[2], p[2], q[3])));
        const float d = (float)(x - xlo);
        if (d < 0.f) return QO_SIDE - 1 - qo_side_bucket(-d * side_w);
        if (d > span_w) return QO_SIDE + QO_MID + qo_side_bucket((d - span_w) * side_w);
        const float f = d * (float)scale;
        return QO_SIDE + (f > 0.f ? (f < (float)(QO_MID - 1) ? (int)f : QO_MID - 1) : 0);
    };
    __syncthreads();
    float rk_lo = 0.f, rk_hi = 0.f, rk_side = 0.f;
    if (ranked) {
        int jl = 0, jh = mt - 1;
        if (mt >= 3 && lkeys[mt - 1] - lkeys[mt - 2] > lkeys[mt - 2] - lkeys[0]) jh = mt - 2;
        if (mt >= 3 && lkeys[1] - lkeys[0] > lkeys[jh] - lkeys[1]) jl = 1;
        rk_lo = lkeys[jl]; rk_hi = lkeys[jh];
        rk_side = rk_hi > rk_lo ? (float)QO_SIDE / (rk_hi - rk_lo) : 0.f;
    }
    constexpr int PER = 16;
    int bk[PER], rk[PER];
    const bool small = n <= PER * QO_THREADS;
    if (small && ranked) {
        float xq[PER];
#pragma unroll
        for (int e = 0; e < PER; ++e) {
            const int i = min(e * QO_THREADS + tid, n - 1);
            const T* p = src + ((size_t)cloud * n + i) * 3;
            xq[e] = (float)fma_t(q[0], p[0], fma_t(q[1], p[1], fma_t(q[2], p[2], q[3])));
        }
#pragma unroll
        for (int e = 0; e < PER; ++e) {
            const int i = e * QO_THREADS + tid;
            int bb = -1, rr = 0;
            if (i < n) {
                const float x = xq[e];
                float f = (x - (float)xlo) * (float)tscale;
                f = f > 0.f ? (f < (float)nbkt_range ? f : (float)nbkt_range) : 0.f;
                const int tb = (int)f;
                int lo = ltab[tb], hi = ltab[min(tb + 1, nbkt_range)];
                if (!(lo <= hi) || (lo > 0 && !(lkeys[lo - 1] < x)) || (hi < mt && lkeys[hi] < x)) { lo = 0; hi = mt; }
                while (lo < hi) { const int mid = (lo + hi) >> 1; if (lkeys[mid] < x) lo = mid + 1; else hi = mid; }
                if (x < rk_lo) bb = QO_SIDE - 1 - qo_side_bucket((rk_lo - x) * rk_side);
// ... 180 lines not shown
```

### dicp_amd/csrc/knn_f16.hip

```cpp
#include <stdlib.h>
#include <type_traits>

#include "dicp_common.h"
#include "dicp_internal.h"
#include "dicp_fill.h"

namespace {

typedef _Float16 half8 __attribute__((ext_vector_type(8)));
typedef float f32x16 __attribute__((ext_vector_type(16)));

constexpr int F16_META = dicp_tu::KNN_F16_META;
constexpr int F16_STAGE = dicp_tu::KNN_F16_STAGE_ROWS / 32;
constexpr int F16_G = 4;
constexpr int F16_CHT = 4;
constexpr int F16_FAR_MAX = 64;
constexpr int F16_NTC = 8;
#ifndef DICP_F16_SCAN_MAX
#define DICP_F16_SCAN_MAX 6
#endif
constexpr int F16_SCAN_MAX = DICP_F16_SCAN_MAX;
enum { FM_S = 0, FM_INV_S2 = 1, FM_PHI = 2, FM_NFAR = 3, FM_HPHI = 4, FM_FAR_ABOVE = 5, FM_AGAIN = 6 ,
       FM_SCAN = 7 , FM_FAR0 = 8 };
constexpr float F16_P = 8192.f;
constexpr float F16_U = 5.9604644775390625e-8f;
constexpr float F16_CREL = 32.f;

__device__ __forceinline__ int f16_row_of(int rho) { return ((rho >> 2) & 1) * 16 + (rho >> 3) * 4 + (rho & 3); }

constexpr int F16_SCALE_THREADS = 1024;
__device__ __forceinline__ float block_max(float v, float* red) {
#pragma unroll
    for (int o = WAVE / 2; o > 0; o >>= 1) v = fmaxf(v, __shfl_xor(v, o));
    __syncthreads();
    if ((threadIdx.x & (WAVE - 1)) == 0) red[threadIdx.x >> 6] = v;
    __syncthreads();
    float r = red[0];
    for (int w = 1; w < F16_SCALE_THREADS / WAVE; ++w) r = fmaxf(r, red[w]);
    return r;
}

struct FormPick {
    const int32_t* tally; const int32_t* src_rows; int n_full, tiles, dflt;
};
__device__ __forceinline__ bool form_long(const FormPick& f, int cloud) {
    if (!f.tally) return true;
    const int t = f.tally[cloud], units = (rows_of(f.src_rows, cloud, f.n_full) + 32 * F16_G - 1) / (32 * F16_G);
    return t > 0 ? t > f.tiles * units : f.dflt != 0;
}

__global__ __launch_bounds__(F16_SCALE_THREADS) void knn_f16_scale_kernel(const float4* __restrict__ rows4, const int32_t* __restrict__ tgt_rows, int m_full, int m_pad,
                                                              float* __restrict__ meta_all) {
    __shared__ float red[F16_SCALE_THREADS / WAVE];
    __shared__ int s_cnt;
    const int cloud = blockIdx.x, tid = threadIdx.x;
    const int m = min(max(rows_of(tgt_rows, cloud, m_full), 1), m_pad);
    const float4* __restrict__ tg = rows4 + (size_t)cloud * m_pad;
    float* mt = meta_all + (size_t)cloud * F16_META;
    int32_t* mi = (int32_t*)mt;
    auto row_max = [&](int r) {
        const float4 v = tg[r];
        return (v.w < __builtin_huge_valf()) ? fmaxf(fmaxf(fabsf(v.x), fabsf(v.y)), fabsf(v.z)) : -1.f;
    };
    auto repeats = [&](int r) {
        if (r == 0) return false;
        const float4 v = tg[r], p = tg[r - 1];
        return __float_as_uint(v.x) == __float_as_uint(p.x) && __float_as_uint(v.y) == __float_as_uint(p.y) && __float_as_uint(v.z) == __float_as_uint(p.z) &&
               __float_as_uint(v.w) == __float_as_uint(p.w);
    };
    float mx = 0.f;
    for (int r = tid; r < m; r += F16_SCALE_THREADS) mx = fmaxf(mx, row_max(r));
    const float Minf = block_max(mx, red);
    if (tid == 0) s_cnt = 0;
    __syncthreads();
    const float cut = Minf * 0.0625f;
    float m2 = 0.f;
    int above = 0;
    for (int r = tid; r < m; r += F16_SCALE_THREADS) { const float v = row_max(r); if (v > cut) above += repeats(r) ? 0 : 1; else m2 = fmaxf(m2, v); }
    if (above) atomicAdd(&s_cnt, above);
    const float M2 = block_max(m2, red);
    const int cnt = s_cnt;
    __syncthreads();
    const bool use_far = cnt > 0 && cnt <= F16_FAR_MAX && M2 > 0.f && cnt * 64 <= m;
    const float M = use_far ? M2 : Minf;
    if (tid == 0) s_cnt = 0;
    __syncthreads();
    if (use_far)
        for (int r = tid; r < m; r += F16_SCALE_THREADS)
            if (row_max(r) > cut && !repeats(r)) { const int slot = atomicAdd(&s_cnt, 1); if (slot < F16_FAR_MAX) mi[FM_FAR0 + slot] = r; }
    __syncthreads();
    if (tid == 0) {
        int ex = 0;
        float s = 1.f;
        if (M > 0.f && M < __builtin_huge_valf()) {
            (void)frexpf(M, &ex);
            const int e = min(max(11 - ex, -60), 60);
            s = ldexpf(1.f, e);
        }
        mt[FM_S] = s;
        mt[FM_INV_S2] = (1.f / s) * (1.f / s);
        mt[FM_PHI] = F16_U / s;
        mi[FM_NFAR] = use_far ? min(s_cnt, F16_FAR_MAX) : 0;
        mt[FM_HPHI] = 3.f * 0.000244140625f * ((1.f / s) * (1.f / s));
        mt[FM_FAR_ABOVE] = use_far ? cut : __builtin_huge_valf();
        mi[FM_AGAIN] = mi[FM_SCAN] = 0;
    }
}

__global__ __launch_bounds__(BLOCK) void knn_f16_image_kernel(const float4* __restrict__ rows4, const int32_t* __restrict__ tgt_rows, int m_full, int m_pad, int m_img,
                                                              const float* __restrict__ meta_all, uint4* __restrict__ image, int tiles_per_cloud, int N,
                                                              float* __restrict__ edges ) {
    const int cloud = blockIdx.y;
    const int tile = blockIdx.x * (BLOCK / WAVE) + (threadIdx.x >> 6), lane = threadIdx.x & (WAVE - 1);
    if (tile >= tiles_per_cloud) return;
    const int m = min(max(rows_of(tgt_rows, cloud, m_full), 1), m_pad);
    const float* mt = meta_all + (size_t)cloud * F16_META;
    const float s = mt[FM_S], far_above = mt[FM_FAR_ABOVE];
    const int r = tile * 32 + f16_row_of(lane & 31), kh = lane >> 5;
    if (kh == 0 && r < m_pad && (r & 63) == 0) edges[((size_t)cloud * (tiles_per_cloud / 2) + (r >> 6)) * 2] = rows4[(size_t)cloud * m_pad + r].x;
    if (kh == 0 && r < m_pad && (r & 63) == 63) edges[((size_t)cloud * (tiles_per_cloud / 2) + (r >> 6)) * 2 + 1] = rows4[(size_t)cloud * m_pad + r].x;
    _Float16 yh[3] = {0, 0, 0}, yl[3] = {0, 0, 0}, H[3] = {(_Float16)__builtin_huge_valf(), 0, 0};
    if (r < m) {
        const float4 v = rows4[(size_t)cloud * m_pad + r];
        const float big = fmaxf(fmaxf(fabsf(v.x), fabsf(v.y)), fabsf(v.z));
        if (v.w < __builtin_huge_valf() && !(big > far_above)) {
            const float c[3] = {v.x * s, v.y * s, v.z * s};
#pragma unroll
            for (int k = 0; k < 3; ++k) { yh[k] = (_Float16)c[k]; yl[k] = (_Float16)(c[k] - (float)yh[k]); }
            const float hs = v.w * (s * s * (1.f / F16_P));
            H[0] = (_Float16)hs;
            const float r1 = hs - (float)H[0];
            H[1] = (_Float16)r1;
            H[2] = (_Float16)(r1 - (float)H[1]);
        }
    }
    half8 a;
    if (kh == 0) { a[0] = yh[0]; a[1] = yh[1]; a[2] = yh[2]; a[3] = yl[0]; a[4] = yl[1]; a[5] = yl[2]; a[6] = yh[0]; a[7] = yh[1]; }
    else         { a[0] = yh[2]; a[1] = yl[0]; a[2] = yl[1]; a[3] = yl[2]; a[4] = H[0];  a[5] = H[1];  a[6] = H[2];  a[7] = (_Float16)0.f; }
    uint4 out;
    __builtin_memcpy(&out, &a, 16);
    image[((size_t)cloud * tiles_per_cloud + tile) * 64 + lane] = out;
}

__device__ __forceinline__ half8 f16_query_fragment(const float* nx, float s, int kh, bool& ok) {
    _Float16 xh[3], xl[3];
    ok = true;
#pragma unroll
    for (int k = 0; k < 3; ++k) {
        float c = nx[k] * s;
        if (!(fabsf(c) <= 60000.f)) { ok = false; c = 0.f; }
        xh[k] = (_Float16)c; xl[k] = (_Float16)(c - (float)xh[k]);
    }
    if (!ok) { xh[0] = xh[1] = xh[2] = xl[0] = xl[1] = xl[2] = (_Float16)0.f; }
    half8 b;
    const _Float16 P = (_Float16)F16_P;
    if (kh == 0) { b[0] = xh[0]; b[1] = xh[1]; b[2] = xh[2]; b[3] = xh[0]; b[4] = xh[1]; b[5] = xh[2]; b[6] = xl[0]; b[7] = xl[1]; }
    else         { b[0] = xl[2]; b[1] = xl[0]; b[2] = xl[1]; b[3] = xl[2]; b[4] = P;     b[5] = P;     b[6] = P;     b[7] = (_Float16)0.f; }
    return b;
}

__device__ __forceinline__ float f16_sqrt_up(float v) { return __builtin_amdgcn_sqrtf(v) * 1.00001f + 1e-18f; }

__device__ __forceinline__ float f16_margin(const float* nx, float b1, float s, float inv_s2, float phi, float hphi) {
    const float x1 = fabsf(nx[0]) + fabsf(nx[1]) + fabsf(nx[2]);
    const float hx = 0.5f * (nx[0] * nx[0] + nx[1] * nx[1] + nx[2] * nx[2]);
    const float b1u = b1 * inv_s2;
    const float D0 = fmaxf(b1u + hx, 0.f);
    const float slack = 0.001953125f * (D0 + hx);
    const float Dup = D0 + slack;
    const float X2 = f16_sqrt_up(2.f * hx);
    const float Y = X2 + f16_sqrt_up(2.f * Dup);
    const float Tup = X2 * Y + 0.5f * Y * Y;
    const float E = (F16_CREL * F16_U * Tup + phi * (x1 + 1.7321f * Y) + hphi) * 1.01f;
    if (!(4.f * E <= slack) || !(E < __builtin_huge_valf())) return -1.f;
    return 2.f * E * (s * s) * 1.0001f;
}
__device__ __forceinline__ float f16_margin(const float* nx, float b1, const float* __restrict__ mt) {
    return f16_margin(nx, b1, mt[FM_S], mt[FM_INV_S2], mt[FM_PHI], mt[FM_HPHI]);
}

__device__ __forceinline__ unsigned swap32(unsigned v) {
    const auto r = __builtin_amdgcn_permlane32_swap(v, v, false, false);
    return (threadIdx.x & 32) ? r[0] : r[1];
}
__device__ __forceinline__ float swap32(float v) { return __uint_as_float(swap32(__float_as_uint(v))); }
__device__ __forceinline__ int swap32(int v) { return (int)swap32((unsigned)v); }

__device__ __forceinline__ float vmin(float a, float b) { float r; asm("v_min_f32 %0, %1, %2" : "=v"(r) : "v"(a), "v"(b)); return r; }
__device__ __forceinline__ float vmax(float a, float b) { float r; asm("v_max_f32 %0, %1, %2" : "=v"(r) : "v"(a), "v"(b)); return r; }

__device__ __forceinline__ float f16_chunk_min(const f32x16& d, float cm) {
#pragma unroll
    for (int i = 0; i < 16; i += 2) cm = __builtin_fminf(__builtin_fminf(cm, d[i]), d[i + 1]);
    return cm;
}

struct F16Track {
    float b1, b2, b3;
    int id1, id2;
    __device__ __forceinline__ void init() { b1 = b2 = b3 = __builtin_huge_valf(); id1 = id2 = 0; }
    __device__ __forceinline__ void add(float cm, int chunk ) {
        asm("v_cmp_lt_f32 vcc, %5, %1\n\t"
            "v_cndmask_b32 %4, %4, %6, vcc\n\t"
            "v_cmp_lt_f32 vcc, %5, %0\n\t"
            "v_cndmask_b32 %4, %4, %3, vcc\n\t"
            "v_cndmask_b32 %3, %3, %6, vcc\n\t"
            "v_med3_f32 %2, %1, %5, %2\n\t"
            "v_med3_f32 %1, %0, %5, %1\n\t"
            "v_min_f32 %0, %0, %5"
            : "+v"(b1), "+v"(b2), "+v"(b3), "+v"(id1), "+v"(id2) : "v"(cm), "v"(chunk) : "vcc");
    }
};

static_assert(F16_STAGE * 64 / BLOCK == 4, "DICP_F16_FETCH / _COMMIT move four 16-byte pieces per thread");
#define DICP_F16_FETCH(st_)  { const uint4* f_ = img + (size_t)(st_) * (F16_STAGE * 64) + tid; pre0 = f_[0]; pre1 = f_[BLOCK]; pre2 = f_[2 * BLOCK]; pre3 = f_[3 * BLOCK]; }
#define DICP_F16_COMMIT(buf_) { uint4* c_ = &lds[buf_][tid]; c_[0] = pre0; c_[BLOCK] = pre1; c_[2 * BLOCK] = pre2; c_[3 * BLOCK] = pre3; }

template <int MINW>
__global__ __launch_bounds__(BLOCK, MINW) void knn_f16_kernel(const float* __restrict__ src, const float* __restrict__ pose, const float4* __restrict__ tgt4,
                                                              const uint4* __restrict__ image, float* __restrict__ meta_all, int32_t* __restrict__ idx,
                                                              int N, int n_full, int m_full, int m_pad_full, int tiles_per_cloud, int bpc,
                                                              const int32_t* __restrict__ src_rows, const int32_t* __restrict__ tgt_rows) {
    __shared__ uint4 lds[2][F16_STAGE * 64];
    __shared__ float4 qlist[BLOCK / WAVE][32];
    __shared__ int qslot[BLOCK / WAVE][32];
    __shared__ int s_rounds;
    int cloud, blk;
    if (!decode_block(bpc, N, cloud, blk)) return;
    const int tid = threadIdx.x, lane = tid & (WAVE - 1), wave = tid >> 6;
    const int n = rows_of(src_rows, cloud, n_full), m = min(max(rows_of(tgt_rows, cloud, m_full), 1), m_pad_full);
    if (blk * (BLOCK / WAVE) * (32 * F16_G) >= n) return;
    const int col = lane & 31, kh = lane >> 5;
    const int qwave = (blk * (BLOCK / WAVE) + wave) * (32 * F16_G);
    float* __restrict__ mt = meta_all + (size_t)cloud * F16_META;
    const float s = mt[FM_S];
    float C[9], r[3];
    load_pose(pose, cloud, C, r);
    if (tid == 0) s_rounds = 0;

    float nx[F16_G][3];
    F16Track tr[F16_G];
    half8 b[F16_G];
    int q_ok = 0;
#pragma unroll
    for (int g = 0; g < F16_G; ++g) {
        const int i = qwave + g * 32 + col;
        float p[3] = {0.f, 0.f, 0.f};
        if (i < n) {
            const float* sp = src + ((size_t)cloud * n_full + i) * 3;
            p[0] = sp[0]; p[1] = sp[1]; p[2] = sp[2];
        }
        query_point(C, r, p, nx[g]);
        bool ok;
        b[g] = f16_query_fragment(nx[g], s, kh, ok);
        q_ok |= ok ? (1 << g) : 0;
        tr[g].init();
    }

    const uint4* __restrict__ img = image + (size_t)cloud * tiles_per_cloud * 64;
    const int nst = (m + 32 * F16_STAGE - 1) / (32 * F16_STAGE);
    f32x16 zero;
#pragma unroll
    for (int i = 0; i < 16; ++i) zero[i] = 0.f;
    uint4 pre0, pre1, pre2, pre3;
    DICP_F16_FETCH(0)
    DICP_F16_COMMIT(0)
    __syncthreads();
    for (int st = 0; st < nst; ++st) {
        const int cur = st & 1;
        if (st + 1 < nst) { DICP_F16_FETCH(st + 1) }
#pragma unroll 1
        for (int t = 0; t < F16_STAGE; t += F16_CHT) {
            half8 a[F16_CHT];
#pragma unroll
            for (int c = 0; c < F16_CHT; ++c) { const uint4 v = lds[cur][(t + c) * 64 + lane]; __builtin_memcpy(&a[c], &v, 16); }
            int chunk = st * (F16_STAGE / F16_CHT) + t / F16_CHT;
            asm("v_mov_b32 %0, %1" : "=v"(chunk) : "s"(chunk));
#pragma unroll
            for (int g = 0; g < F16_G; ++g) {
                float cm = __builtin_huge_valf();
#pragma unroll
                for (int c = 0; c < F16_CHT; ++c)
                    cm = f16_chunk_min(__builtin_amdgcn_mfma_f32_32x32x16_f16(a[c], b[g], zero, 0, 0, 0), cm);
                tr[g].add(cm, chunk);
            }
        }
        if (st + 1 < nst) { DICP_F16_COMMIT(cur ^ 1) }
        __syncthreads();
    }

    const float4* __restrict__ tg = tgt4 + (size_t)cloud * m_pad_full;
    const int nfar = ((const int32_t*)mt)[FM_NFAR];
    float bv[F16_G], thr[F16_G];
// ... 518 lines not shown
                put_best(slot >> 8, col == (slot & 0xff), r);
            }
            __builtin_amdgcn_wave_barrier();
        }
    }

    if (nfar > 0) {
#pragma unroll 1
        for (int g = 0; g < F16_G; ++g) {
            float qq[3];
#pragma unroll
            for (int k = 0; k < 3; ++k) qq[k] = g == 0 ? nx[0][k] : (g == 1 ? nx[1][k] : (g == 2 ? nx[2][k] : nx[3][k]));
            SweepBest w;
            w.v = DICP_PICK4(bV, g); w.s = DICP_PICK4(bS, g); w.o = DICP_PICK4(bO, g);
#pragma unroll 1
            for (int f = 0; f < nfar; ++f) {
                const int rr = ((const int32_t*)mt)[FM_FAR0 + f];
                if (rr < m) sweep_consider(w, qq, tg[rr], rr, pm);
            }
            put_best(g, true, w);
        }
    }
#pragma unroll
    for (int g = 0; g < F16_G; ++g) {
        if (qi[g] < 0 || kh != 0) continue;
        const bool found = bV[g] < __builtin_huge_valf();
        int bo = bO[g];
        if (found && bo < 0) bo = pm[bS[g]];
        if (!found) bo = 0x7fffffff;
        if (idx) idx[(size_t)cloud * n_full + qi[g]] = (bo == 0x7fffffff) ? 0 : min(max(bo, 0), m - 1);
        if (spos) spos[(size_t)cloud * n_full + qi[g]] = (bo == 0x7fffffff || bo >= m) ? -1 : bS[g];
    }
    if (lane == 0) {
        if (cnt) atomicAdd((int*)mt + FM_AGAIN, cnt);
        if (n_scan) atomicAdd((int*)mt + FM_SCAN, n_scan);
        if (pairs) atomicAdd(pairs + (blockIdx.x & (DICP_PAIR_SHARDS - 1)), (unsigned long long)(visR - visL) * WAVE * (32 * F16_G));
        if (form_out) atomicAdd(form_out + cloud, visR - visL);
    }
}
#undef DICP_PICK4

template <int MINW>
__global__ __launch_bounds__(BLOCK, MINW) void knn_f16_sweep_kernel(const float* __restrict__ src, const float* __restrict__ pose, const float4* __restrict__ tgs4,
                                                                    const uint4* __restrict__ image, float* __restrict__ meta_all,
                                                                    const int32_t* __restrict__ tperm, const int32_t* __restrict__ qorder,
                                                                    const int32_t* __restrict__ bucket, const float* __restrict__ brange, int nbkt,
                                                                    int32_t* __restrict__ idx, int32_t* __restrict__ spos, unsigned long long* __restrict__ pairs,
                                                                    int N, int n_full, int m_full, int m_pad, int tiles_per_cloud, int bpc,
                                                                    const int32_t* __restrict__ src_rows, const int32_t* __restrict__ tgt_rows,
                                                                    const float* __restrict__ edges_all, FormPick pick, int32_t* __restrict__ form_out) {
    int cloud, blk;
    if (!decode_block(bpc, N, cloud, blk)) return;
    if (!form_long(pick, cloud)) return;
    f16_sweep_unit(src, pose, tgs4, image, meta_all, tperm, qorder, bucket, brange, nbkt, idx, spos, pairs, N, n_full, m_full, m_pad, tiles_per_cloud, bpc,
                   src_rows, tgt_rows, edges_all, form_out, cloud, blk);
}

__global__ __launch_bounds__(BLOCK) void knn_f16_probe_kernel(const float* __restrict__ src, const float* __restrict__ pose, const float4* __restrict__ tgt4,
                                                               const uint4* __restrict__ image, const float* __restrict__ meta_all, int N, int n_full, int m_full,
                                                               int m_pad, int tiles_per_cloud, int bpc, const int32_t* __restrict__ src_rows,
                                                               const int32_t* __restrict__ tgt_rows, float* __restrict__ out ) {
    int cloud, blk;
    if (!decode_block(bpc, N, cloud, blk)) return;
    const int lane = threadIdx.x & (WAVE - 1), wave = threadIdx.x >> 6, col = lane & 31, kh = lane >> 5;
    const int n = rows_of(src_rows, cloud, n_full), m = min(max(rows_of(tgt_rows, cloud, m_full), 1), m_pad);
    const int q = (blk * (BLOCK / WAVE) + wave) * 32 + col;
    if ((blk * (BLOCK / WAVE) + wave) * 32 >= n) return;
    const float* mt = meta_all + (size_t)cloud * F16_META;
    const float s = mt[FM_S], inv_s2 = mt[FM_INV_S2], phi = mt[FM_PHI], hphi = mt[FM_HPHI];
    float C[9], r[3];
    load_pose(pose, cloud, C, r);
    float p[3] = {0.f, 0.f, 0.f}, nx[3];
    if (q < n) { const float* sp = src + ((size_t)cloud * n_full + q) * 3; p[0] = sp[0]; p[1] = sp[1]; p[2] = sp[2]; }
    query_point(C, r, p, nx);
    bool ok;
    const half8 b = f16_query_fragment(nx, s, kh, ok);
    ok = ok && q < n;
    const float x1 = fabsf(nx[0]) + fabsf(nx[1]) + fabsf(nx[2]);
    const float4* __restrict__ tg = tgt4 + (size_t)cloud * m_pad;
    const uint4* __restrict__ img = image + (size_t)cloud * tiles_per_cloud * 64;
    f32x16 zero;
#pragma unroll
    for (int i = 0; i < 16; ++i) zero[i] = 0.f;
    double best = 0.0, best_err = 0.0, best_E = 0.0;
    unsigned long long cnt = 0;
    const int ntiles = min((m + 31) / 32, tiles_per_cloud);
    for (int t = 0; t < ntiles; ++t) {
        half8 a;
        { const uint4 v = img[(size_t)t * 64 + lane]; __builtin_memcpy(&a, &v, 16); }
        const f32x16 d = __builtin_amdgcn_mfma_f32_32x32x16_f16(a, b, zero, 0, 0, 0);
#pragma unroll
        for (int i = 0; i < 16; ++i) {
            const int row = t * 32 + 16 * kh + i;
            const float f = d[i];
            if (!ok || row >= m || !(f < __builtin_huge_valf()) || !(f > -__builtin_huge_valf())) continue;
            const float4 y = tg[row];
            const float sc = score<float, float4>(nx, y);
            const double err = fabs((double)f * (double)inv_s2 - (double)sc);
            const double T = fabs((double)nx[0] * y.x) + fabs((double)nx[1] * y.y) + fabs((double)nx[2] * y.z) + (double)y.w;
            const double ynorm = sqrt(2.0 * (double)y.w);
            const double E = (double)F16_CREL * (double)F16_U * T + (double)phi * ((double)x1 + 1.7321 * ynorm) + (double)hphi;
            const double ratio = err / E;
            ++cnt;
            if (ratio > best) { best = ratio; best_err = err; best_E = E; }
        }
    }
#pragma unroll 1
    for (int o = WAVE / 2; o > 0; o >>= 1) {
        const double ob = __shfl_xor(best, o), oe = __shfl_xor(best_err, o), oE = __shfl_xor(best_E, o);
        cnt += __shfl_xor(cnt, o);
        if (ob > best) { best = ob; best_err = oe; best_E = oE; }
    }
    if (lane == 0) {
        const float bf = (float)best;
        const int old = atomicMax((int*)out + (size_t)cloud * 4, __float_as_int(bf));
        if (__float_as_int(bf) > old) { out[(size_t)cloud * 4 + 1] = (float)best_err; out[(size_t)cloud * 4 + 2] = (float)best_E; }
        atomicAdd(out + (size_t)cloud * 4 + 3, (float)cnt);
    }
}

}

namespace dicp_tu {

int knn_f16_probe(const void* src, const void* pose, const void* tgt4, const void* image, const int32_t* src_rows, const int32_t* tgt_rows,
                  int N, int n, int m, int m_pad, float* out, void* stream) {
    if (!src || !tgt4 || !image || !out) return DICP_ERR_NULL;
    if (N <= 0 || n <= 0 || m <= 0 || m_pad < m) return DICP_ERR_SHAPE;
    hipStream_t st = (hipStream_t)stream;
    const int m_img = knn_f16_image_rows(m_pad), tiles = m_img / 32;
    const float* meta = (const float*)((const char*)image + knn_f16_meta_offset(N, m_pad));
    const int bpc = (n + (BLOCK / WAVE) * 32 - 1) / ((BLOCK / WAVE) * 32);
    begin_launch();
    if (const int e = dicp_fill::zero(out, (size_t)N * 4 * sizeof(float), st)) return e;
    knn_f16_probe_kernel<<<grid_for(N, bpc), BLOCK, 0, st>>>((const float*)src, (const float*)pose, (const float4*)tgt4, (const uint4*)image, meta, N, n, m, m_pad, tiles, bpc,
                                                             src_rows, tgt_rows, out);
    return launch_status();
}

int knn_f16_pack(const void* rows4, const int32_t* tgt_rows, int N, int m_full, int m_pad, void* image, void* stream) {
    if (!rows4 || !image) return DICP_ERR_NULL;
    if (N <= 0 || m_full <= 0 || m_pad < m_full || (m_pad % 32)) return DICP_ERR_SHAPE;
    if (((uintptr_t)rows4 % 16) || ((uintptr_t)image % 16)) return DICP_ERR_ALIGN;
    hipStream_t st = (hipStream_t)stream;
    const int m_img = knn_f16_image_rows(m_pad), tiles = m_img / 32;
    float* meta = (float*)((char*)image + knn_f16_meta_offset(N, m_pad));
    float* edges = (float*)((char*)image + knn_f16_edges_offset(N, m_pad));
    begin_launch();
    knn_f16_scale_kernel<<<N, F16_SCALE_THREADS, 0, st>>>((const float4*)rows4, tgt_rows, m_full, m_pad, meta);
    knn_f16_image_kernel<<<dim3((tiles + BLOCK / WAVE - 1) / (BLOCK / WAVE), N), BLOCK, 0, st>>>((const float4*)rows4, tgt_rows, m_full, m_pad, m_img, meta, (uint4*)image, tiles, N, edges);
    return launch_status();
}

int knn_f16_brute(const void* src, const void* pose, const void* tgt4, void* image, const int32_t* src_rows, const int32_t* tgt_rows,
                  int N, int n, int m, int m_pad, int32_t* idx, void* stream) {
    if (!src || !tgt4 || !image || !idx) return DICP_ERR_NULL;
    if (N <= 0 || n <= 0 || m <= 0 || m_pad < m) return DICP_ERR_SHAPE;
    hipStream_t st = (hipStream_t)stream;
    const int m_img = knn_f16_image_rows(m_pad), tiles = m_img / 32;
    float* meta = (float*)((char*)image + knn_f16_meta_offset(N, m_pad));
    const int bpc = (n + (BLOCK / WAVE) * 32 * F16_G - 1) / ((BLOCK / WAVE) * 32 * F16_G);
    begin_launch();
    knn_f16_kernel<4><<<grid_for(N, bpc), BLOCK, 0, st>>>((const float*)src, (const float*)pose, (const float4*)tgt4, (const uint4*)image, meta, idx,
                                                         N, n, m, m_pad, tiles, bpc, src_rows, tgt_rows);
    return launch_status();
}

int knn_f16_sweep(const void* src, const void* pose, const void* tgs4, void* image, const int32_t* tperm, const int32_t* qorder, const int32_t* bucket,
                  const void* brange, int nbkt, const int32_t* src_rows, const int32_t* tgt_rows, int N, int n, int m, int m_pad, int32_t* idx, int32_t* spos,
                  unsigned long long* pairs, const int32_t* form_in, int32_t* form_out, int form_tiles, int form_default, void* ev0, void* ev1, void* stream) {
    if (!src || !tgs4 || !image || !tperm || !bucket || !brange || (!idx && !spos)) return DICP_ERR_NULL;
    if (N <= 0 || n <= 0 || m <= 0 || m_pad < m || (m_pad % WAVE)) return DICP_ERR_SHAPE;
    const int m_img = knn_f16_image_rows(m_pad), tiles = m_img / 32;
    float* meta = (float*)((char*)image + knn_f16_meta_offset(N, m_pad));
    const float* edges = (const float*)((const char*)image + knn_f16_edges_offset(N, m_pad));
    const int units = (n + 32 * F16_G - 1) / (32 * F16_G);
    const int bpc = (units + BLOCK / WAVE - 1) / (BLOCK / WAVE);
    const FormPick pick{form_in, src_rows, n, form_tiles, form_default};
    begin_launch();
    hipExtLaunchKernelGGL((knn_f16_sweep_kernel<4>), dim3(grid_for(N, bpc)), dim3(BLOCK), 0, (hipStream_t)stream, (hipEvent_t)ev0, (hipEvent_t)ev1, 0,
                          (const float*)src, (const float*)pose, (const float4*)tgs4, (const uint4*)image, meta, tperm, qorder, bucket, (const float*)brange, nbkt,
                          idx, spos, pairs, N, n, m, m_pad, tiles, bpc, src_rows, tgt_rows, edges, pick, form_out);
    return launch_status();
}

}
```

### include/dicp_hip.h

```cpp
#ifndef DICP_HIP_H
#define DICP_HIP_H
#include <stddef.h>
#include <stdint.h>

#ifdef __cplusplus
extern "C" {
#endif

#define DICP_ABI_VERSION 11

enum { DICP_F32 = 0, DICP_F64 = 1 };
enum { DICP_PT2PT = 0, DICP_PT2PL = 1 };
enum { DICP_LOSS_NONE = 0, DICP_LOSS_HUBER = 1, DICP_LOSS_CAUCHY = 2, DICP_LOSS_TRIM = 3 };
enum { DICP_KNN_AUTO = 0, DICP_KNN_VALU = 1, DICP_KNN_MFMA = 2, DICP_KNN_SWEEP = 3 ,
       DICP_KNN_GUMBEL = 4  };
enum { DICP_ERR_NULL = 1, DICP_ERR_SHAPE = 2, DICP_ERR_DTYPE = 3, DICP_ERR_ENUM = 4, DICP_ERR_ALIGN = 5, DICP_ERR_ABI = 6  };

#define DICP_NACC_PAD 32
#define DICP_NBWD_PAD 16

typedef struct dicp_weight_params {
    int32_t mode;
    int32_t trim_on;
    int32_t differentiable;
    int32_t loss;
    double trim_dist;
    double tanh_k;
    double loss_delta;
    double match_thresh;
} dicp_weight_params;

int dicp_abi_version(void);
int dicp_copy(void* dst, const void* src, size_t bytes, void* stream);
int dicp_zero(void* dst, size_t bytes, void* stream);

int dicp_padded_targets(int m);
int dicp_accumulate_blocks(int n);

int dicp_search_frame(int dtype, const void* tgt, int c, const int32_t* tgt_rows, int N, int m, double quantum, int directions,
                      const void* src, const int32_t* src_rows, int n, const void* T_init, void* frame, void* stream);

int dicp_pack_target(int dtype, const void* tgt, int c, const void* frame, const int32_t* tgt_rows, int N, int m, void* tgt4, int m_pad, void* stream);

size_t dicp_knn_f16_bytes(int N, int m_pad);
int dicp_knn_f16_pack(const void* tgt4, const int32_t* tgt_rows, int N, int m, int m_pad, void* image, void* stream);
int dicp_knn_f16_probe(const void* src, const void* pose, const void* tgt4, const void* f16_image, const int32_t* src_rows, const int32_t* tgt_rows,
                       int N, int n, int m, int m_pad, float* out, void* stream);

int dicp_knn(int dtype, const void* src, const void* pose, const void* tgt4, const int32_t* src_rows, const int32_t* tgt_rows,
             int N, int n, int m, int m_pad, int32_t* idx, int variant, const void* f16_image, void* stream);

size_t dicp_sweep_sort_scratch_bytes(int dtype, int N, int m_pad);
int dicp_sweep_sort(int dtype, const void* tgt, int c, const void* frame, const int32_t* tgt_rows, int N, int m, int m_pad, void* keys_sorted,
                    int32_t* tperm, int nbkt, int32_t* bucket, void* brange, void* scratch, size_t scratch_bytes, void* stream);
int dicp_sweep_build(int dtype, const void* tgt, int c, const void* frame, const int32_t* tgt_rows, const int32_t* tperm, int N, int m, int m_pad,
                     void* tgs4, void* tgt_s, int tgt_s_stride, void* stream);
int dicp_sweep_setup(int dtype, const void* tgt, int c, const int32_t* tgt_rows, int N, int m, int m_pad, double quantum, int directions,
                     void* frame, void* keys_sorted, int32_t* tperm, int nbkt, int32_t* bucket, void* brange, void* scratch, size_t scratch_bytes,
                     void* tgs4, void* tgt_s, int tgt_s_stride,
                     const void* src, const int32_t* src_rows, int n, const void* T_init, void* pose_search0, int32_t* qorder0, void* stream);

int dicp_query_keys(int dtype, const void* src, const void* pose, int N, int n, void* keys, void* stream);
int dicp_query_order(int dtype, const void* src, const void* pose, const void* brange, int nbkt, int N, int n, int32_t* qorder,
                     const void* w, void* src_s, void* w_s, int reproducible, const int32_t* spos_prev, int m_pad,
                     const void* keys_sorted, const int32_t* bucket, int m, const int32_t* src_rows, const int32_t* tgt_rows, void* stream);
int dicp_query_reorder(int dtype, const void* src, const void* pose, const void* pose_prev, const int32_t* order_prev, const void* brange, int nbkt, int N, int n,
                       int32_t* qorder, int m_pad, const void* skeys, const int32_t* bucket, int m, const int32_t* src_rows, const int32_t* tgt_rows, void* stream);

#define DICP_PAIR_SHARDS 64
int dicp_knn_sweep(int dtype, const void* src, const void* pose, const void* tgs4, const int32_t* tperm,
                   const int32_t* qorder, const int32_t* bucket, const void* brange, int nbkt, const int32_t* src_rows, const int32_t* tgt_rows,
                   int N, int n, int m, int m_pad, int32_t* idx, int32_t* spos, unsigned long long* pairs, int cfg, const void* f16_image,
                   const int32_t* form_in, int32_t* form_out, int form_default, void* stream);

int dicp_gather_rows(int dtype, const void* tgt, const int32_t* idx, int N, int n, int m, int c, void* out, void* stream);
int dicp_pack_list(int dtype, const void* const* ptrs, const int32_t* lens, const int32_t* strides, int N, int n_max, int cols, void* out, const void* pad, void* stream);
int dicp_unpack_list(int dtype, const void* gout, void* const* ptrs, const int32_t* lens, const int32_t* strides, int N, int n_max, int cols, int stride_max, void* stream);
int dicp_scatter_add_rows(int dtype, const void* gout, const int32_t* idx, int N, int n, int m, int c, void* gtgt, void* stream);

int dicp_accumulate(int dtype, const dicp_weight_params* prm, const void* src, const void* tgt, int c,
                    const int32_t* idx, const void* pose, const void* w_init, const void* alive, const int32_t* src_rows,
                    int N, int n, int m, void* partials, void* w_out, int64_t w_stride, void* stream);

typedef struct dicp_step_io {
    const void* partials;
    int32_t nblk;
    int32_t iter;
    int32_t dim;
    int32_t const_iter;
    double tolerance;
    int32_t rows_per_point;
    int32_t n;
    const void* pose_in;
    void* pose_out;
    void* delta;
    int64_t delta_stride;
    void* cost;
    const void* cost_prev;
    int64_t cost_stride;
    double* areg;
    const void* alive;
    void* alive_out;
    uint8_t* converged;
    void* iterations;
    void* matched_ratio;
    const void* n_start;
    void* n_matched;
    void* w_cur;
    const void* w_prev;
    int64_t w_stride;
    int32_t* n_not_converged;
    const void* frame;
    void* pose_search_out;
    const void* rmax;
    void* dcum;
    int64_t dcum_stride;
    int32_t* cert_cloud;
    const void* cert_qu;
    int32_t cert_units;
    int32_t glist_cap;
    int32_t* glist;
    int32_t* gcount;
    int32_t* cert_scount;
    int32_t* cert_slist;
    int32_t w_copied;
} dicp_step_io;

int dicp_step(int dtype, const dicp_step_io* io, int N, void* stream);

typedef struct dicp_gumbel_loop {
    const void* const* U;
    const uint32_t* seeds;
    double eps, tau;
    void* ps_t;
    void* nbr;
    void* lse;
    void* g_nbr;
    void* g_ps;
} dicp_gumbel_loop;

typedef struct dicp_search_buffers {
    int32_t knn_variant;
    int32_t m_pad;
    const void* tgt4;
    const int32_t* tperm;
    const int32_t* qorder;
    const int32_t* bucket;
    const void* brange;
    int32_t nbkt;
    unsigned long long* pairs;
    const void* frame;
    void* poses;
    const void* tgt_sorted;
    int32_t tgt_sorted_stride;
    const dicp_gumbel_loop* gumbel;
    int32_t first_done;
    const void* tgt_f16;
    int32_t* form;
    int32_t form_default;
    const int32_t* form_plan;
} dicp_search_buffers;

typedef struct dicp_cert_buffers {
    void* q;
    void* qu;
    void* set;
    int32_t* count;
    void* rmax;
    void* dcum;
    int32_t reset;
    int32_t* cloud;
    void* nbr;
    int32_t* gdirty;
    int32_t* pend;
    int32_t* glist;
    int32_t* gcount;
    int32_t* slist;
    int32_t* scount;
    int32_t* cm;
} dicp_cert_buffers;

typedef struct dicp_history_buffers {
    int32_t per_iter;
    int32_t* spos;
    void* poses;
    void* deltas;
    void* costs;
    double* areg;
    void* alive;
    int32_t* idx;
    void* w;
    int64_t w_iter, w_stride;
    const void* w_prev0;
    const int32_t* spos_prev_chunk;
    int32_t spos_floor;
    int32_t* spos_of;
    int32_t spos_of_from;
} dicp_history_buffers;

typedef struct dicp_bwd_buffers {
    const int32_t* spos_ref;
    void* gts_far;
    int32_t overwrite;
    int32_t* skip;
    double* mref;
    int32_t* live;
    double skip_eps;
    int32_t tail_from;
    void* tail_partials;
    int32_t* tail_arrive;
    int32_t* det_far_row;
    void* det_far_val;
} dicp_bwd_buffers;
// ... 357 lines not shown
```

Before: 3.312 million.

## Fuse f16 target-image metadata and first search pose into sweep setup kernels

Adds a combined sweep setup entry point. The sort-keys kernel now also computes the f16 image scale/far-row metadata, and the search-frame kernel writes the initial search pose directly. The f16 image is built right after the sorted rows, so the separate scale-pass kernel and the pose-composition launch are no longer needed. This trims per-call setup launches and target passes, at the cost of more shared memory and a larger sort kernel in the META variant.

```diff
diff --git a/dicp_amd/_lib.py b/dicp_amd/_lib.py
--- a/dicp_amd/_lib.py
+++ b/dicp_amd/_lib.py
@@ -7,7 +7,7 @@
 _ROOT = os.path.dirname(_HERE)
 LIB_PATH = os.environ.get("DICP_HIP_LIB") or os.path.join(_HERE, "libdicp_hip.so")
 SOURCES = [os.path.join(_HERE, "csrc", f) for f in ("dicp_kernels.hip", "knn_f16.hip", "dicp_call.hip", "normals.hip", "voxel.hip", "knn_points.hip", "fps.hip", "ball_query.hip", "knn_grid.hip", "group.hip", "inverse.hip", "knn_det.hip", "normals_det.hip", "filter.hip")]
-HEADERS = ([os.path.join(_HERE, "csrc", f) for f in ("dicp_math.h", "dicp_common.h", "dicp_internal.h", "dicp_fill.h", "dicp_normals.h", "dicp_voxel.h", "dicp_topk.h", "dicp_fps.h", "dicp_ball.h", "dicp_gridknn.h", "kernels_grid.h", "kernels_grid_plan.h", "dicp_group.h", "dicp_group_launch.h", "dicp_inverse.h", "dicp_knn_det.h", "kernels_normals.h", "dicp_normals_det.h", "dicp_filter.h")]
+HEADERS = ([os.path.join(_HERE, "csrc", f) for f in ("dicp_math.h", "dicp_common.h", "dicp_internal.h", "dicp_f16_image.h", "dicp_fill.h", "dicp_normals.h", "dicp_voxel.h", "dicp_topk.h", "dicp_fps.h", "dicp_ball.h", "dicp_gridknn.h", "kernels_grid.h", "kernels_grid_plan.h", "dicp_group.h", "dicp_group_launch.h", "dicp_inverse.h", "dicp_knn_det.h", "kernels_normals.h", "dicp_normals_det.h", "dicp_filter.h")]
            + [os.path.join(_HERE, "csrc", "kernels_%s.h" % f) for f in ("setup", "search", "setup_sort", "rows", "accumulate", "backward", "soft_svd", "host")]
            + [os.path.join(_ROOT, "include", "dicp_hip.h")])
 
@@ -169,6 +169,7 @@
     "dicp_sweep_sort": ([i32, vp, i32, vp, vp, i32, i32, i32, vp, vp, i32, vp, vp, vp, ctypes.c_size_t, vp], ctypes.c_int),
     "dicp_sweep_build": ([i32, vp, i32, vp, vp, vp, i32, i32, i32, vp, vp, i32, vp], ctypes.c_int),
     "dicp_sweep_setup": ([i32, vp, i32, vp, i32, i32, i32, f64, i32, vp, vp, vp, i32, vp, vp, vp, ctypes.c_size_t, vp, vp, i32, vp, vp, i32, vp, vp, vp, vp], ctypes.c_int),
+    "dicp_sweep_setup_f16": ([i32, vp, i32, vp, i32, i32, i32, f64, i32, vp, vp, vp, i32, vp, vp, vp, ctypes.c_size_t, vp, vp, i32, vp, vp, i32, vp, vp, vp, vp, vp], ctypes.c_int),
     "dicp_query_order": ([i32, vp, vp, vp, i32, i32, i32, vp, vp, vp, vp, i32, vp, i32, vp, vp, i32, vp, vp, vp], ctypes.c_int),
     "dicp_query_reorder": ([i32, vp, vp, vp, vp, vp, i32, i32, i32, vp, i32, vp, vp, i32, vp, vp, vp], ctypes.c_int),
     "dicp_query_keys": ([i32, vp, vp, i32, i32, vp, vp], ctypes.c_int),
diff --git a/dicp_amd/_ops.py b/dicp_amd/_ops.py
--- a/dicp_amd/_ops.py
+++ b/dicp_amd/_ops.py
@@ -195,12 +195,12 @@
             self.frame = torch.empty((N, 12), dtype=dt, device=dev)
             pose_s = torch.empty((N, 12), dtype=dt, device=dev)
             qorder = torch.empty((N, source.shape[1]), dtype=torch.int32, device=dev)
+            if want_img:
+                self.img16 = torch.empty((int(lib.dicp_knn_f16_bytes(N, m_pad)),), dtype=torch.uint8, device=dev)
             with _on(dev):
-                _lib.check(lib.dicp_sweep_setup(_DT[dt], _p(tgt), c, _p(tgt_rows), N, m, m_pad, CENTER_QUANTUM, int(FRAME_DIRECTIONS), _p(self.frame), _p(self.keys), _p(self.tperm),
-                                                self.NBKT, _p(self.bucket), _p(self.brange), _p(scratch), nbytes, _p(self.tgs4), _p(self.tgt_s), self.row_stride,
-                                                _p(source), _p(src_rows), source.shape[1], _p(T_init), _p(pose_s), _p(qorder), _stream()), "dicp_sweep_setup")
-            if want_img:
-                self.img16 = f16_image(self.tgs4, m, tgt_rows)
+                _lib.check(lib.dicp_sweep_setup_f16(_DT[dt], _p(tgt), c, _p(tgt_rows), N, m, m_pad, CENTER_QUANTUM, int(FRAME_DIRECTIONS), _p(self.frame), _p(self.keys), _p(self.tperm),
+                                                    self.NBKT, _p(self.bucket), _p(self.brange), _p(scratch), nbytes, _p(self.tgs4), _p(self.tgt_s), self.row_stride,
+                                                    _p(source), _p(src_rows), source.shape[1], _p(T_init), _p(pose_s), _p(qorder), _p(self.img16), _stream()), "dicp_sweep_setup_f16")
             spos0 = None
             if first_search:
                 spos0 = torch.empty((N, source.shape[1]), dtype=torch.int32, device=dev)
diff --git a/dicp_amd/csrc/dicp_f16_image.h b/dicp_amd/csrc/dicp_f16_image.h
--- /dev/null
+++ b/dicp_amd/csrc/dicp_f16_image.h
@@ -0,0 +1,82 @@
+#pragma once
+#include <hip/hip_runtime.h>
+
+#include "dicp_common.h"
+#include "dicp_internal.h"
+
+namespace dicp_f16 {
+
+typedef _Float16 half8 __attribute__((ext_vector_type(8)));
+
+constexpr int F16_META = dicp_tu::KNN_F16_META;
+constexpr int F16_FAR_MAX = 64;
+enum { FM_S = 0, FM_INV_S2 = 1, FM_PHI = 2, FM_NFAR = 3, FM_HPHI = 4, FM_FAR_ABOVE = 5, FM_AGAIN = 6 ,
+       FM_SCAN = 7 , FM_FAR0 = 8 };
+constexpr float F16_P = 8192.f;
+constexpr float F16_U = 5.9604644775390625e-8f;
+
+__device__ __forceinline__ int f16_row_of(int rho) { return ((rho >> 2) & 1) * 16 + (rho >> 3) * 4 + (rho & 3); }
+
+__device__ __forceinline__ float f16_row_big(const float4& v) {
+    return (v.w < __builtin_huge_valf()) ? fmaxf(fmaxf(fabsf(v.x), fabsf(v.y)), fabsf(v.z)) : -1.f;
+}
+__device__ __forceinline__ bool f16_same_row(const float4& v, const float4& p) {
+    return __float_as_uint(v.x) == __float_as_uint(p.x) && __float_as_uint(v.y) == __float_as_uint(p.y) && __float_as_uint(v.z) == __float_as_uint(p.z) &&
+           __float_as_uint(v.w) == __float_as_uint(p.w);
+}
+
+template <int THREADS>
+__device__ __forceinline__ float f16_block_max(float v, float* red) {
+#pragma unroll
+    for (int o = WAVE / 2; o > 0; o >>= 1) v = fmaxf(v, __shfl_xor(v, o));
+    __syncthreads();
+    if ((threadIdx.x & (WAVE - 1)) == 0) red[threadIdx.x >> 6] = v;
+    __syncthreads();
+    float r = red[0];
+    for (int w = 1; w < THREADS / WAVE; ++w) r = fmaxf(r, red[w]);
+    return r;
+}
+
+__device__ __forceinline__ bool f16_use_far(int cnt, float M2, int m) { return cnt > 0 && cnt <= F16_FAR_MAX && M2 > 0.f && cnt * 64 <= m; }
+
+__device__ __forceinline__ void f16_write_meta(float* __restrict__ mt, float M, bool use_far, int nfar, float cut) {
+    int32_t* mi = (int32_t*)mt;
+    int ex = 0;
+    float s = 1.f;
+    if (M > 0.f && M < __builtin_huge_valf()) {
+        (void)frexpf(M, &ex);
+        const int e = min(max(11 - ex, -60), 60);
+        s = ldexpf(1.f, e);
+    }
+    mt[FM_S] = s;
+    mt[FM_INV_S2] = (1.f / s) * (1.f / s);
+    mt[FM_PHI] = F16_U / s;
+    mi[FM_NFAR] = use_far ? min(nfar, F16_FAR_MAX) : 0;
+    mt[FM_HPHI] = 3.f * 0.000244140625f * ((1.f / s) * (1.f / s));
+    mt[FM_FAR_ABOVE] = use_far ? cut : __builtin_huge_valf();
+    mi[FM_AGAIN] = mi[FM_SCAN] = 0;
+}
+
+__device__ __forceinline__ void f16_row_pieces(const float4& v, bool real, float s, float far_above, uint4& p0, uint4& p1) {
+    _Float16 yh[3] = {0, 0, 0}, yl[3] = {0, 0, 0}, H[3] = {(_Float16)__builtin_huge_valf(), 0, 0};
+    if (real) {
+        const float big = fmaxf(fmaxf(fabsf(v.x), fabsf(v.y)), fabsf(v.z));
+        if (v.w < __builtin_huge_valf() && !(big > far_above)) {
+            const float c[3] = {v.x * s, v.y * s, v.z * s};
+#pragma unroll
+            for (int k = 0; k < 3; ++k) { yh[k] = (_Float16)c[k]; yl[k] = (_Float16)(c[k] - (float)yh[k]); }
+            const float hs = v.w * (s * s * (1.f / F16_P));
+            H[0] = (_Float16)hs;
+            const float r1 = hs - (float)H[0];
+            H[1] = (_Float16)r1;
+            H[2] = (_Float16)(r1 - (float)H[1]);
+        }
+    }
+    half8 a, b;
+    a[0] = yh[0]; a[1] = yh[1]; a[2] = yh[2]; a[3] = yl[0]; a[4] = yl[1]; a[5] = yl[2]; a[6] = yh[0]; a[7] = yh[1];
+    b[0] = yh[2]; b[1] = yl[0]; b[2] = yl[1]; b[3] = yl[2]; b[4] = H[0];  b[5] = H[1];  b[6] = H[2];  b[7] = (_Float16)0.f;
+    __builtin_memcpy(&p0, &a, 16);
+    __builtin_memcpy(&p1, &b, 16);
+}
+
+}
diff --git a/dicp_amd/csrc/dicp_internal.h b/dicp_amd/csrc/dicp_internal.h
--- a/dicp_amd/csrc/dicp_internal.h
+++ b/dicp_amd/csrc/dicp_internal.h
@@ -11,6 +11,7 @@
 inline size_t knn_f16_meta_offset(int N, int m_pad) { return (size_t)N * knn_f16_image_rows(m_pad) * 32; }
 inline size_t knn_f16_edges_offset(int N, int m_pad) { return knn_f16_meta_offset(N, m_pad) + (size_t)N * KNN_F16_META * 4; }
 int knn_f16_pack(const void* rows4, const int32_t* tgt_rows, int N, int m_full, int m_pad, void* image, void* stream);
+int knn_f16_image(const void* rows4, const int32_t* tgt_rows, int N, int m_full, int m_pad, void* image, void* stream);
 int knn_f16_probe(const void* src, const void* pose, const void* tgt4, const void* image, const int32_t* src_rows, const int32_t* tgt_rows,
                   int N, int n, int m, int m_pad, float* out, void* stream);
 int knn_f16_brute(const void* src, const void* pose, const void* tgt4, void* image, const int32_t* src_rows, const int32_t* tgt_rows,
diff --git a/dicp_amd/csrc/dicp_kernels.hip b/dicp_amd/csrc/dicp_kernels.hip
--- a/dicp_amd/csrc/dicp_kernels.hip
+++ b/dicp_amd/csrc/dicp_kernels.hip
@@ -5,6 +5,7 @@
 #include "dicp_common.h"
 #include "dicp_internal.h"
 #include "dicp_fill.h"
+#include "dicp_f16_image.h"
 
 namespace {
 
@@ -75,7 +76,7 @@
     hipStream_t st = (hipStream_t)stream;
     if (dtype == DICP_F32 && m_pad <= RS_MAX) {
         begin_launch();
-        sort_keys_kernel<<<N, RS_THREADS, 0, st>>>((const float*)tgt, c, N, m, m_pad, (float*)keys_sorted, tperm, nbkt, bucket, (float*)brange, (const float*)frame, tgt_rows);
+        sort_keys_kernel<false><<<N, RS_THREADS, 0, st>>>((const float*)tgt, c, N, m, m_pad, (float*)keys_sorted, tperm, nbkt, bucket, (float*)brange, (const float*)frame, tgt_rows);
         return launch_status();
     }
     if (!scratch || scratch_bytes < dicp_sweep_sort_scratch_bytes(dtype, N, m_pad)) return DICP_ERR_NULL;
@@ -127,6 +128,42 @@
         if (!rc) rc = dicp_query_order(dtype, src, pose_search0, brange, nbkt, N, n, qorder0, nullptr, nullptr, nullptr, 0, nullptr, m_pad, keys_sorted, bucket, m,
                                        src_rows, tgt_rows, stream);
     }
+    return rc;
+}
+
+int dicp_sweep_setup_f16(int dtype, const void* tgt, int c, const int32_t* tgt_rows, int N, int m, int m_pad, double quantum, int directions,
+                         void* frame, void* keys_sorted, int32_t* tperm, int nbkt, int32_t* bucket, void* brange, void* scratch, size_t scratch_bytes,
+                         void* tgs4, void* tgt_s, int tgt_s_stride,
+                         const void* src, const int32_t* src_rows, int n, const void* T_init, void* pose_search0, int32_t* qorder0, void* f16_image, void* stream) {
+    if (f16_image && dtype != DICP_F32) return DICP_ERR_DTYPE;
+    if (dtype != DICP_F32 || m_pad > RS_MAX) {
+        int rc = dicp_sweep_setup(dtype, tgt, c, tgt_rows, N, m, m_pad, quantum, directions, frame, keys_sorted, tperm, nbkt, bucket, brange, scratch, scratch_bytes,
+                                  tgs4, tgt_s, tgt_s_stride, src, src_rows, n, T_init, pose_search0, qorder0, stream);
+        if (!rc && f16_image) rc = dicp_tu::knn_f16_pack(tgs4, tgt_rows, N, m, m_pad, f16_image, stream);
+        return rc;
+    }
+    if (!tgt || !frame || !keys_sorted || !tperm || (bucket && !brange) || !tgs4) return DICP_ERR_NULL;
+    if (bucket && nbkt <= 0) return DICP_ERR_SHAPE;
+    if (N <= 0 || m <= 0 || (c != 3 && c != 6) || !(quantum >= 0.0) || (src && T_init && n <= 0) || m_pad != dicp_padded_targets(m) || (tgt_s && tgt_s_stride < c)) return DICP_ERR_SHAPE;
+    if (((uintptr_t)tgs4 % 16) || ((uintptr_t)f16_image % 16)) return DICP_ERR_ALIGN;
+    const bool first = T_init && pose_search0 && qorder0;
+    if (first && (!src || n <= 0)) return DICP_ERR_NULL;
+    const void* T_pose = T_init;
+    if (!src || !T_init) { src = nullptr; T_init = nullptr; }
+    hipStream_t st = (hipStream_t)stream;
+    begin_launch();
+    search_frame_kernel<float><<<N, CC_THREADS, 0, st>>>((const float*)tgt, c, m, tgt_rows, quantum, directions, (float*)frame, (const float*)src, n, src_rows, (const float*)T_init,
+                                                         first ? (const float*)T_pose : nullptr, first ? (float*)pose_search0 : nullptr);
+    float* meta = f16_image ? (float*)((char*)f16_image + dicp_tu::knn_f16_meta_offset(N, m_pad)) : nullptr;
+    if (meta) sort_keys_kernel<true><<<N, RS_THREADS, 0, st>>>((const float*)tgt, c, N, m, m_pad, (float*)keys_sorted, tperm, nbkt, bucket, (float*)brange, (const float*)frame, tgt_rows, meta);
+    else      sort_keys_kernel<false><<<N, RS_THREADS, 0, st>>>((const float*)tgt, c, N, m, m_pad, (float*)keys_sorted, tperm, nbkt, bucket, (float*)brange, (const float*)frame, tgt_rows);
+    const int bpc = (m_pad + BLOCK * 4 - 1) / (BLOCK * 4);
+    sweep_rows_kernel<float><<<grid_for(N, bpc), BLOCK, 0, st>>>((const float*)tgt, tgt_rows, N, m, c, m_pad, bpc, (float4*)tgs4, tperm, (float*)tgt_s, tgt_s_stride, (const float*)frame);
+    int rc = launch_status();
+    if (!rc && f16_image) rc = dicp_tu::knn_f16_image(tgs4, tgt_rows, N, m, m_pad, f16_image, stream);
+    if (!rc && first)
+        rc = dicp_query_order(dtype, src, pose_search0, brange, nbkt, N, n, qorder0, nullptr, nullptr, nullptr, 0, nullptr, m_pad, keys_sorted, bucket, m,
+                              src_rows, tgt_rows, stream);
     return rc;
 }
 
diff --git a/dicp_amd/csrc/kernels_setup.h b/dicp_amd/csrc/kernels_setup.h
--- a/dicp_amd/csrc/kernels_setup.h
+++ b/dicp_amd/csrc/kernels_setup.h
@@ -40,7 +40,9 @@
 template <typename T>
 __global__ __launch_bounds__(CC_THREADS) void search_frame_kernel(const T* __restrict__ tgt, int c, int m, const int32_t* __restrict__ tgt_rows,
                                                                   double quantum, int directions, T* __restrict__ frame,
-                                                                  const T* __restrict__ src, int n, const int32_t* __restrict__ src_rows, const T* __restrict__ T_init) {
+                                                                  const T* __restrict__ src, int n, const int32_t* __restrict__ src_rows, const T* __restrict__ T_init,
+                                                                  const T* __restrict__ T_pose = nullptr ,
+                                                                  T* __restrict__ pose_search0 = nullptr ) {
     const double QS[SF_DIRS][9] = {
         {1, 0, 0, 0, 1, 0, 0, 0, 1}, {0, 1, 0, 0, 0, 1, 1, 0, 0}, {0, 0, 1, 1, 0, 0, 0, 1, 0},
         {0.6, 0.64, 0.48, 0.72953720414008516, -0.68394112888132985, 0, 0.32829174186303833, 0.35017785798724088, -0.87726848797845247},
@@ -54,6 +56,7 @@
     __shared__ int s_cost[SF_DIRS];
     __shared__ float4 s_t[CC_SAMPLE];
     __shared__ int s_cum[SF_DIRS][256 + 1];
+    __shared__ T s_F[12];
     const int cloud = blockIdx.x, tid = threadIdx.x, lane = tid & (WAVE - 1), wave = tid >> 6;
     const T* __restrict__ rows = tgt + (size_t)cloud * m * c;
     const int mc = max(rows_of(tgt_rows, cloud, m), 1);
@@ -204,12 +207,23 @@
     }
     if (tid < 12) {
         T* F = frame + (size_t)cloud * 12;
-        if (tid < 9) F[tid] = (T)QS[best][tid];
+        T f;
+        if (tid < 9) f = (T)QS[best][tid];
         else {
             const int i = tid - 9;
             const T cx = (T)s_ctr[0], cy = (T)s_ctr[1], cz = (T)s_ctr[2];
-            F[tid] = best == 0 ? -(i == 0 ? cx : (i == 1 ? cy : cz))
-                               : -fma_t((T)QS[best][3 * i], cx, fma_t((T)QS[best][3 * i + 1], cy, (T)QS[best][3 * i + 2] * cz));
+            f = best == 0 ? -(i == 0 ? cx : (i == 1 ? cy : cz))
+                          : -fma_t((T)QS[best][3 * i], cx, fma_t((T)QS[best][3 * i + 1], cy, (T)QS[best][3 * i + 2] * cz));
+        }
+        F[tid] = f;
+        s_F[tid] = f;
+    }
+    if (pose_search0 && T_pose) {
+        __syncthreads();
+        if (tid < 12) {
+            const T* M = T_pose + (size_t)cloud * 16;
+            const T ps[12] = {M[0], M[1], M[2], M[4], M[5], M[6], M[8], M[9], M[10], M[3], M[7], M[11]};
+            pose_search0[(size_t)cloud * 12 + tid] = frame_pose_entry<T>(s_F, ps, tid);
         }
     }
 }
@@ -296,26 +310,57 @@
     u ^= (u >> 31) ? 0xffffffffu : 0x80000000u;
     return x != x ? 0xffffffffu : u;
 }
+template <bool META = false>
 __global__ __launch_bounds__(RS_THREADS) void sort_keys_kernel(const float* __restrict__ tgt, int c, int N, int m_full, int m_pad,
                                                                float* __restrict__ keys_sorted, int32_t* __restrict__ tperm,
                                                                int nbkt, int32_t* __restrict__ bucket, float* __restrict__ brange,
-                                                               const float* __restrict__ frame, const int32_t* __restrict__ tgt_rows) {
+                                                               const float* __restrict__ frame, const int32_t* __restrict__ tgt_rows,
+                                                               float* __restrict__ meta_all = nullptr) {
     __shared__ unsigned skey[RS_MAX];
     __shared__ unsigned short sidx[RS_MAX];
     __shared__ int cnt[RS_THREADS / WAVE][256];
     __shared__ int tot[256];
+    __shared__ unsigned farbits[META ? RS_MAX / 32 : 1];
+    __shared__ int farlist[META ? dicp_f16::F16_FAR_MAX : 1];
+    __shared__ float red[RS_THREADS / WAVE];
+    __shared__ int s_far;
+    __shared__ float s_ext[2];
     const int cloud = blockIdx.x, tid = threadIdx.x, lane = tid & (WAVE - 1), wave = tid >> 6;
     const float* __restrict__ rows = tgt + (size_t)cloud * m_full * c;
     const int m = rows_of(tgt_rows, cloud, m_full);
     unsigned key[RS_PER];
     unsigned short idx[RS_PER];
+    [[maybe_unused]] float mx = 0.f;
 #pragma unroll
     for (int e = 0; e < RS_PER; ++e) {
         const int pos = wave * (WAVE * RS_PER) + e * WAVE + lane;
         unsigned u = 0xffffffffu;
-        if (pos < m) { float q[3]; frame_apply<float>(frame ? frame + (size_t)cloud * 12 : nullptr, rows + (size_t)pos * c, q); u = sortable_bits(q[0]); }
+        if constexpr (META) {
+            float big = -1.f;
+            if (pos < m) { const float4 v = pack_row<float>(rows + (size_t)pos * c, frame ? frame + (size_t)cloud * 12 : nullptr); u = sortable_bits(v.x); big = dicp_f16::f16_row_big(v); }
+            skey[pos] = __float_as_uint(big);
+            mx = fmaxf(mx, big);
+        } else {
+            if (pos < m) { float q[3]; frame_apply<float>(frame ? frame + (size_t)cloud * 12 : nullptr, rows + (size_t)pos * c, q); u = sortable_bits(q[0]); }
+        }
         key[e] = u;
         idx[e] = (unsigned short)pos;
+    }
+    if constexpr (META) {
+        const float Minf = dicp_f16::f16_block_max<RS_THREADS>(mx, red);
+        const float cut = Minf * 0.0625f;
+        float m2 = 0.f;
+        if (tid == 0) s_far = 0;
+#pragma unroll
+        for (int e = 0; e < RS_PER; ++e) {
+            const float big = __uint_as_float(skey[wave * (WAVE * RS_PER) + e * WAVE + lane]);
+            const bool far = big > cut;
+            const unsigned long long bal = __ballot(far);
+            if (lane == 0) { farbits[wave * (WAVE * RS_PER / 32) + 2 * e] = (unsigned)bal; farbits[wave * (WAVE * RS_PER / 32) + 2 * e + 1] = (unsigned)(bal >> 32); }
+            if (!far) m2 = fmaxf(m2, big);
+        }
+        const float M2 = dicp_f16::f16_block_max<RS_THREADS>(m2, red);
+        if (tid == 0) { s_ext[0] = Minf; s_ext[1] = M2; }
     }
     for (int pass = 0; pass < 4; ++pass) {
         const int shift = pass * 8;
@@ -373,15 +418,51 @@
         }
         __syncthreads();
     }
+    int lane_t = lane, wave_t = wave;
+    if constexpr (META) {
+        asm volatile("" : "+v"(lane_t));
+        wave_t = __builtin_amdgcn_readfirstlane(wave);
+    }
 #pragma unroll
     for (int e = 0; e < RS_PER; ++e) {
-        const int pos = wave * (WAVE * RS_PER) + e * WAVE + lane;
+        const int pos = wave_t * (WAVE * RS_PER) + e * WAVE + lane_t;
         if (pos < m_pad) {
             unsigned u = key[e];
             u ^= (u >> 31) ? 0x80000000u : 0xffffffffu;
             keys_sorted[(size_t)cloud * m_pad + pos] = __uint_as_float(u);
             tperm[(size_t)cloud * m_pad + pos] = (int32_t)idx[e];
         }
+    }
+    if constexpr (META) {
+        const float* F = frame ? frame + (size_t)cloud * 12 : nullptr;
+        auto far_row = [&](int e, int pos) {
+            const int o = idx[e];
+            if (pos >= m || !((farbits[o >> 5] >> (o & 31)) & 1u)) return false;
+            if (pos == 0 || skey[pos - 1] != key[e]) return true;
+            return !dicp_f16::f16_same_row(pack_row<float>(rows + (size_t)o * c, F), pack_row<float>(rows + (size_t)sidx[pos - 1] * c, F));
+        };
+        int above = 0;
+#pragma unroll
+        for (int e = 0; e < RS_PER; ++e) above += __popcll(__ballot(far_row(e, wave_t * (WAVE * RS_PER) + e * WAVE + lane_t)));
+        if (lane_t == 0 && above) atomicAdd(&s_far, above);
+        __syncthreads();
+        const int nfar = s_far, m_rows = min(max(m, 1), m_pad);
+        const float Minf = s_ext[0], M2 = s_ext[1];
+        const bool use_far = dicp_f16::f16_use_far(nfar, M2, m_rows);
+        __syncthreads();
+        float* mt = meta_all + (size_t)cloud * dicp_f16::F16_META;
+        if (use_far) {
+            if (tid == 0) s_far = 0;
+            __syncthreads();
+#pragma unroll
+            for (int e = 0; e < RS_PER; ++e) {
+                const int pos = wave_t * (WAVE * RS_PER) + e * WAVE + lane_t;
+                if (far_row(e, pos)) { const int slot = atomicAdd(&s_far, 1); if (slot < dicp_f16::F16_FAR_MAX) farlist[slot] = pos; }
+            }
+            __syncthreads();
+            if (tid < min(nfar, dicp_f16::F16_FAR_MAX)) ((int32_t*)mt)[dicp_f16::FM_FAR0 + tid] = farlist[tid];
+        }
+        if (tid == 0) dicp_f16::f16_write_meta(mt, use_far ? M2 : Minf, use_far, nfar, Minf * 0.0625f);
     }
     if (bucket) {
         auto key_at = [&](int i) { unsigned u = skey[i]; u ^= (u >> 31) ? 0x80000000u : 0xffffffffu; return __uint_as_float(u); };
diff --git a/dicp_amd/csrc/knn_f16.hip b/dicp_amd/csrc/knn_f16.hip
--- a/dicp_amd/csrc/knn_f16.hip
+++ b/dicp_amd/csrc/knn_f16.hip
@@ -4,41 +4,26 @@
 #include "dicp_common.h"
 #include "dicp_internal.h"
 #include "dicp_fill.h"
+#include "dicp_f16_image.h"
 
 namespace {
 
-typedef _Float16 half8 __attribute__((ext_vector_type(8)));
+using namespace dicp_f16;
+
 typedef float f32x16 __attribute__((ext_vector_type(16)));
 
-constexpr int F16_META = dicp_tu::KNN_F16_META;
 constexpr int F16_STAGE = dicp_tu::KNN_F16_STAGE_ROWS / 32;
 constexpr int F16_G = 4;
 constexpr int F16_CHT = 4;
-constexpr int F16_FAR_MAX = 64;
 constexpr int F16_NTC = 8;
 #ifndef DICP_F16_SCAN_MAX
 #define DICP_F16_SCAN_MAX 6
 #endif
 constexpr int F16_SCAN_MAX = DICP_F16_SCAN_MAX;
-enum { FM_S = 0, FM_INV_S2 = 1, FM_PHI = 2, FM_NFAR = 3, FM_HPHI = 4, FM_FAR_ABOVE = 5, FM_AGAIN = 6 ,
-       FM_SCAN = 7 , FM_FAR0 = 8 };
-constexpr float F16_P = 8192.f;
-constexpr float F16_U = 5.9604644775390625e-8f;
 constexpr float F16_CREL = 32.f;
 
-__device__ __forceinline__ int f16_row_of(int rho) { return ((rho >> 2) & 1) * 16 + (rho >> 3) * 4 + (rho & 3); }
-
 constexpr int F16_SCALE_THREADS = 1024;
-__device__ __forceinline__ float block_max(float v, float* red) {
-#pragma unroll
-    for (int o = WAVE / 2; o > 0; o >>= 1) v = fmaxf(v, __shfl_xor(v, o));
-    __syncthreads();
-    if ((threadIdx.x & (WAVE - 1)) == 0) red[threadIdx.x >> 6] = v;
-    __syncthreads();
-    float r = red[0];
-    for (int w = 1; w < F16_SCALE_THREADS / WAVE; ++w) r = fmaxf(r, red[w]);
-    return r;
-}
+__device__ __forceinline__ float block_max(float v, float* red) { return f16_block_max<F16_SCALE_THREADS>(v, red); }
 
 struct FormPick {
     const int32_t* tally; const int32_t* src_rows; int n_full, tiles, dflt;
@@ -58,16 +43,8 @@
     const float4* __restrict__ tg = rows4 + (size_t)cloud * m_pad;
     float* mt = meta_all + (size_t)cloud * F16_META;
     int32_t* mi = (int32_t*)mt;
-    auto row_max = [&](int r) {
-        const float4 v = tg[r];
-        return (v.w < __builtin_huge_valf()) ? fmaxf(fmaxf(fabsf(v.x), fabsf(v.y)), fabsf(v.z)) : -1.f;
-    };
-    auto repeats = [&](int r) {
-        if (r == 0) return false;
-        const float4 v = tg[r], p = tg[r - 1];
-        return __float_as_uint(v.x) == __float_as_uint(p.x) && __float_as_uint(v.y) == __float_as_uint(p.y) && __float_as_uint(v.z) == __float_as_uint(p.z) &&
-               __float_as_uint(v.w) == __float_as_uint(p.w);
-    };
+    auto row_max = [&](int r) { return f16_row_big(tg[r]); };
+    auto repeats = [&](int r) { return r != 0 && f16_same_row(tg[r], tg[r - 1]); };
     float mx = 0.f;
     for (int r = tid; r < m; r += F16_SCALE_THREADS) mx = fmaxf(mx, row_max(r));
     const float Minf = block_max(mx, red);
@@ -81,7 +58,7 @@
     const float M2 = block_max(m2, red);
     const int cnt = s_cnt;
     __syncthreads();
-    const bool use_far = cnt > 0 && cnt <= F16_FAR_MAX && M2 > 0.f && cnt * 64 <= m;
+    const bool use_far = f16_use_far(cnt, M2, m);
     const float M = use_far ? M2 : Minf;
     if (tid == 0) s_cnt = 0;
     __syncthreads();
@@ -89,22 +66,7 @@
         for (int r = tid; r < m; r += F16_SCALE_THREADS)
             if (row_max(r) > cut && !repeats(r)) { const int slot = atomicAdd(&s_cnt, 1); if (slot < F16_FAR_MAX) mi[FM_FAR0 + slot] = r; }
     __syncthreads();
-    if (tid == 0) {
-        int ex = 0;
-        float s = 1.f;
-        if (M > 0.f && M < __builtin_huge_valf()) {
-            (void)frexpf(M, &ex);
-            const int e = min(max(11 - ex, -60), 60);
-            s = ldexpf(1.f, e);
-        }
-        mt[FM_S] = s;
-        mt[FM_INV_S2] = (1.f / s) * (1.f / s);
-        mt[FM_PHI] = F16_U / s;
-        mi[FM_NFAR] = use_far ? min(s_cnt, F16_FAR_MAX) : 0;
-        mt[FM_HPHI] = 3.f * 0.000244140625f * ((1.f / s) * (1.f / s));
-        mt[FM_FAR_ABOVE] = use_far ? cut : __builtin_huge_valf();
-        mi[FM_AGAIN] = mi[FM_SCAN] = 0;
-    }
+    if (tid == 0) f16_write_meta(mt, M, use_far, s_cnt, cut);
 }
 
 __global__ __launch_bounds__(BLOCK) void knn_f16_image_kernel(const float4* __restrict__ rows4, const int32_t* __restrict__ tgt_rows, int m_full, int m_pad, int m_img,
@@ -119,26 +81,9 @@
     const int r = tile * 32 + f16_row_of(lane & 31), kh = lane >> 5;
     if (kh == 0 && r < m_pad && (r & 63) == 0) edges[((size_t)cloud * (tiles_per_cloud / 2) + (r >> 6)) * 2] = rows4[(size_t)cloud * m_pad + r].x;
     if (kh == 0 && r < m_pad && (r & 63) == 63) edges[((size_t)cloud * (tiles_per_cloud / 2) + (r >> 6)) * 2 + 1] = rows4[(size_t)cloud * m_pad + r].x;
-    _Float16 yh[3] = {0, 0, 0}, yl[3] = {0, 0, 0}, H[3] = {(_Float16)__builtin_huge_valf(), 0, 0};
-    if (r < m) {
-        const float4 v = rows4[(size_t)cloud * m_pad + r];
-        const float big = fmaxf(fmaxf(fabsf(v.x), fabsf(v.y)), fabsf(v.z));
-        if (v.w < __builtin_huge_valf() && !(big > far_above)) {
-            const float c[3] = {v.x * s, v.y * s, v.z * s};
-#pragma unroll
-            for (int k = 0; k < 3; ++k) { yh[k] = (_Float16)c[k]; yl[k] = (_Float16)(c[k] - (float)yh[k]); }
-            const float hs = v.w * (s * s * (1.f / F16_P));
-            H[0] = (_Float16)hs;
-            const float r1 = hs - (float)H[0];
-            H[1] = (_Float16)r1;
-            H[2] = (_Float16)(r1 - (float)H[1]);
-        }
-    }
-    half8 a;
-    if (kh == 0) { a[0] = yh[0]; a[1] = yh[1]; a[2] = yh[2]; a[3] = yl[0]; a[4] = yl[1]; a[5] = yl[2]; a[6] = yh[0]; a[7] = yh[1]; }
-    else         { a[0] = yh[2]; a[1] = yl[0]; a[2] = yl[1]; a[3] = yl[2]; a[4] = H[0];  a[5] = H[1];  a[6] = H[2];  a[7] = (_Float16)0.f; }
-    uint4 out;
-    __builtin_memcpy(&out, &a, 16);
+    uint4 p0, p1;
+    f16_row_pieces(r < m ? rows4[(size_t)cloud * m_pad + r] : make_float4(0.f, 0.f, 0.f, 0.f), r < m, s, far_above, p0, p1);
+    const uint4 out = kh == 0 ? p0 : p1;
     image[((size_t)cloud * tiles_per_cloud + tile) * 64 + lane] = out;
 }
 
@@ -963,6 +908,19 @@
     return launch_status();
 }
 
+int knn_f16_image(const void* rows4, const int32_t* tgt_rows, int N, int m_full, int m_pad, void* image, void* stream) {
+    if (!rows4 || !image) return DICP_ERR_NULL;
+    if (N <= 0 || m_full <= 0 || m_pad < m_full || (m_pad % 32)) return DICP_ERR_SHAPE;
+    if (((uintptr_t)rows4 % 16) || ((uintptr_t)image % 16)) return DICP_ERR_ALIGN;
+    hipStream_t st = (hipStream_t)stream;
+    const int m_img = knn_f16_image_rows(m_pad), tiles = m_img / 32;
+    const float* meta = (const float*)((const char*)image + knn_f16_meta_offset(N, m_pad));
+    float* edges = (float*)((char*)image + knn_f16_edges_offset(N, m_pad));
+    begin_launch();
+    knn_f16_image_kernel<<<dim3((tiles + BLOCK / WAVE - 1) / (BLOCK / WAVE), N), BLOCK, 0, st>>>((const float4*)rows4, tgt_rows, m_full, m_pad, m_img, meta, (uint4*)image, tiles, N, edges);
+    return launch_status();
+}
+
 int knn_f16_brute(const void* src, const void* pose, const void* tgt4, void* image, const int32_t* src_rows, const int32_t* tgt_rows,
                   int N, int n, int m, int m_pad, int32_t* idx, void* stream) {
     if (!src || !tgt4 || !image || !idx) return DICP_ERR_NULL;
diff --git a/include/dicp_hip.h b/include/dicp_hip.h
--- a/include/dicp_hip.h
+++ b/include/dicp_hip.h
@@ -59,6 +59,10 @@
                      void* frame, void* keys_sorted, int32_t* tperm, int nbkt, int32_t* bucket, void* brange, void* scratch, size_t scratch_bytes,
                      void* tgs4, void* tgt_s, int tgt_s_stride,
                      const void* src, const int32_t* src_rows, int n, const void* T_init, void* pose_search0, int32_t* qorder0, void* stream);
+int dicp_sweep_setup_f16(int dtype, const void* tgt, int c, const int32_t* tgt_rows, int N, int m, int m_pad, double quantum, int directions,
+                         void* frame, void* keys_sorted, int32_t* tperm, int nbkt, int32_t* bucket, void* brange, void* scratch, size_t scratch_bytes,
+                         void* tgs4, void* tgt_s, int tgt_s_stride,
+                         const void* src, const int32_t* src_rows, int n, const void* T_init, void* pose_search0, int32_t* qorder0, void* f16_image, void* stream);
 
 int dicp_query_keys(int dtype, const void* src, const void* pose, int N, int n, void* keys, void* stream);
 int dicp_query_order(int dtype, const void* src, const void* pose, const void* brange, int nbkt, int N, int n, int32_t* qorder,
```

New measurement: 3.321 million (median of 4 runs). About the same (+0.2%).
